# skycrapers/TecoGAN-PyTorch

Hardware: AMD Instinct MI355X
Metric: HR frames/sec/GPU at 4xSR 3x134x320 LR; Vid4 PSNR vs reference (higher is better)
Workload: dtype f32; 1 GPU; TecoGAN 4xSR BD generator-only inference (FRNet.infer_sequence) of a synthetic 2140-frame 3x134x320 LR clip -> 3x536x1280 HR uint8, 1 clip/GPU, random-init weights (BASELINE configs[1]); a step = one recurrent frame; parallelism=clip-sharded x1, no data-path collective, launches_per_frame=29

## Files before the change

### include/tecogan_hip.h

```cpp
#ifndef TECOGAN_HIP_H
#define TECOGAN_HIP_H

#include <stddef.h>
#include <stdint.h>

#ifdef __cplusplus
extern "C" {
#endif

typedef void* tg_stream_t;

enum {
  TG_OK = 0,
  TG_E_SHAPE = -1,
  TG_E_ARG = -2,
  TG_E_HIP = -3
};

enum {
  TG_ACT_NONE = 0,
  TG_ACT_RELU = 1,
  TG_ACT_LRELU02 = 2,
  TG_ACT_TANH24 = 3
};

enum {
  TG_UP_NONE = 0,
  TG_UP_BICUBIC = 1,
  TG_UP_BILINEAR = 2
};

#define TG_ABI_MAJOR 2
int tg_version(void);
const char* tg_last_error_string(void);
const char* tg_build_info(void);

int tg_conv3x3_pick_ocb(int cout);
size_t tg_conv3x3_packed_floats(int cin, int cout, int ocb);
int tg_conv3x3_pack(const float* w, float* w_packed, int cin, int cout, int ocb,
                    int transposed, tg_stream_t stream);

int tg_conv3x3_fwd(
    const float* x, int64_t x_nstride, int c1,
    const float* x2, int64_t x2_nstride,
    const float* w_packed, int ocb, const float* bias ,
    const float* res, int64_t res_nstride,
    float* y, int64_t y_nstride,
    int n, int cin, int cout, int h, int w, int act, tg_stream_t stream);

int tg_conv3x3_fwd_phased(const float* x, int64_t x_nstride, const float* w_packed, int ocb,
                          const float* bias, float* y, int64_t y_nstride, int n, int cin,
                          int cout, int h, int w, int act, int tapsel, int cphase,
                          int taps_phase0, int taps_phase1, tg_stream_t stream);
int tg_conv4x4s2_supported(int n, int ci, int co, int h, int w);
size_t tg_conv4x4s2_packed_floats(int ci, int co);
int tg_conv4x4s2_pack(const float* w, float* w_fwd, float* w_dgrad, int ci, int co, tg_stream_t stream);
size_t tg_conv4x4s2_workspace_floats(int n, int ci, int co, int h, int w, int dgrad);
int tg_conv4x4s2_fwd(const float* x, const float* w_fwd, float* y, float* workspace, int n, int ci, int co, int h, int w,
                     tg_stream_t stream);
int tg_conv4x4s2_dgrad(const float* g, const float* w_dgrad, const float* act_y, int act, float* dx, float* workspace,
                       int n, int ci, int co, int h, int w, tg_stream_t stream);
int tg_conv3x3s2_supported(int n, int cin, int cout, int h_out, int w_out);
int tg_conv3x3s2_fwd(const float* x, int64_t x_nstride, const float* w_packed, const float* bias,
                     const float* relu_mask, int64_t mask_nstride, float* y, int64_t y_nstride, int n,
                     int cin, int cout, int h_out, int w_out, int act, tg_stream_t stream);
int tg_conv3x3_fwd_phased_masked(const float* x, int64_t x_nstride, const float* w_packed, int ocb,
                                 const float* bias, const float* relu_mask, int64_t mask_nstride,
                                 float* y, int64_t y_nstride, int n, int cin, int cout, int h, int w,
                                 int act, int tapsel, int cphase, int taps_phase0, int taps_phase1,
                                 tg_stream_t stream);
int tg_conv3x3_phased_pick_ksplit(int n, int cin, int cout, int h, int w, int ocb);
int tg_conv3x3_fwd_phased_splitk(const float* x, int64_t x_nstride, const float* w_packed, int ocb,
                                 const float* bias, float* y, int n, int cin, int cout, int h, int w,
                                 int act, int tapsel, int cphase, int taps_phase0, int taps_phase1,
                                 int ksplit, float* partials, tg_stream_t stream);
int tg_conv3x3_fwd_masked(const float* x, int64_t x_nstride, int c1, const float* x2,
                          int64_t x2_nstride, const float* w_packed, int ocb,
                          const float* bias, const float* res, int64_t res_nstride,
                          const float* relu_mask, int64_t mask_nstride, float* y,
                          int64_t y_nstride, int n, int cin, int cout, int h, int w, int act,
                          tg_stream_t stream);

int64_t tg_conv3x3_wino_packed_floats(int cin, int cout);
int tg_conv3x3_prefers_wino(int n, int cin, int cout, int h, int w);
int tg_pack_conv3x3_wino(const float* w, float* out, int cin, int cout, int transposed,
                         tg_stream_t stream);
int tg_conv3x3_wino_fwd(const float* x, int64_t x_nstride, int c1, const float* x2,
                        int64_t x2_nstride, const float* u_packed, const float* bias,
                        const float* res, int64_t res_nstride, const float* relu_mask,
                        int64_t mask_nstride, float* y, int64_t y_nstride, int n, int cin,
                        int cout, int h, int w, int act, tg_stream_t stream);

typedef struct {
  const float* x; const float* x2; const float* u_packed; const float* bias; const float* res;
  float* y;
  int64_t x_nstride, x2_nstride, res_nstride, y_nstride;
  int c1, cin, act;
} tg_wino_layer;
int64_t tg_conv3x3_wino_chain_flag_ints(int n_layers, int n, int h, int w);
int tg_conv3x3_wino_chain(const tg_wino_layer* layers, int n_layers, int n, int cout, int h, int w,
                          int32_t* flags, int epoch, tg_stream_t stream);

int tg_conv3x3_wino_resident_supported(int n, int cout, int h, int w);
int64_t tg_conv3x3_wino_resident_ws_bytes(int h, int w);
int tg_conv3x3_wino_resident(const tg_wino_layer* layers, int n_layers, int cout, int h, int w,
                             void* workspace, int epoch, tg_stream_t stream);
typedef struct tg_wres_convt {
  const float* u_packed;
  const float* bias;
  float* y;
  int act;
} tg_wres_convt;
size_t tg_conv3x3_wino_resident_ct_floats(void);
int tg_conv3x3_wino_resident_ct_pack(const float* w_iohw, float* out, tg_stream_t stream);
int tg_conv3x3_wino_resident_ct(const tg_wino_layer* layers, int n_layers, int cout, int h, int w,
                                void* workspace, int epoch, const tg_wres_convt* convt, tg_stream_t stream);

typedef struct {
  const float* x; const float* x2; const float* w_packed; const float* bias; const float* res;
  const float* relu_mask;
  float* y;
  int64_t x_nstride, x2_nstride, res_nstride, mask_nstride, y_nstride;
  int c1, cin, cout, act;
} tg_chain_layer;
int64_t tg_conv3x3_chain_flag_ints(int n_layers, int n, int h, int w);
int tg_conv3x3_chain_supported(int n, int h, int w, int cmax);
size_t tg_conv3x3_pack16_floats(void);
int tg_conv3x3_pack16(const float* w, float* w_packed, int cin, int cout, int transposed, tg_stream_t stream);
typedef struct tg_pack_item {
  const float* w;
  float* out;
  int cin, cout, transposed, i_total, i_off;
} tg_pack_item;
size_t tg_conv3x3_chain_packed_floats(int pack_layout, int cin);
int tg_conv3x3_chain_pack(const tg_pack_item* items, int n_items, int pack_layout, tg_stream_t stream);
int tg_conv3x3_chain(const tg_chain_layer* layers, int n_layers, int n, int h, int w, int pack_layout,
                     int32_t* flags, int32_t* err, uint32_t epoch, int poll_limit, tg_stream_t stream);
typedef struct { const float* w; const float* b; } tg_packed_layer;
int tg_srnet_body_fwd(const tg_packed_layer* layers, int pack_layout, int nb, const float* lr, int c_lr,
                      const float* tran, int c_tran, float* acts, int n, int nf, int h, int w, int32_t* flags,
                      int32_t* err, uint32_t epoch, int poll_limit, tg_stream_t stream);
int tg_srnet_body_bwd(const tg_packed_layer* dgrad, int pack_layout, int nb, const float* acts, float* dz,
                      float* d_tran, int c_tran, int n, int nf, int h, int w, int32_t* flags, int32_t* err,
                      uint32_t epoch, int poll_limit, tg_stream_t stream);

size_t tg_wgrad3x3_body_workspace_floats(int nframes, int n_per_frame, int nlayers, int c, int h, int w);
int tg_wgrad3x3_body(const float* const* dz_bases, const float* const* act_bases, int nframes, int64_t layer_stride, int nlayers, float* const* grads, float* workspace,
                     int n_per_frame, int c, int h, int w, int accumulate, tg_stream_t stream);
int tg_wgrad3x3_body_bias(const float* const* dz_bases, const float* const* act_bases, int nframes,
                          int64_t layer_stride, int nlayers, float* const* grads, float* const* dbs,
                          float* workspace, int n_per_frame, int c, int h, int w, int accumulate,
                          tg_stream_t stream);
int tg_bias_grad_body(const float* const* dz_bases, int nframes,
                      int64_t layer_stride, int nlayers, float* const* dbs, int n_per_frame, int c, int hw,
                      tg_stream_t stream);

int tg_conv3x3_pick_ksplit(int n, int cin, int cout, int h, int w);
int tg_conv3x3_splitk_fwd(const float* x, int64_t x_nstride, int c1, const float* x2,
                          int64_t x2_nstride, const float* w_packed, int ocb,
                          const float* bias, float* y, int n, int cin, int cout, int h,
                          int w, int act, int ksplit, float* partials, int pool,
                          tg_stream_t stream);

int tg_convt3x3s2_fwd(const float* x, int64_t x_nstride, const float* w_packed,
                      const float* bias, float* y, int64_t y_nstride, int n,
                      int cin, int cout, int h, int w, int act,
                      tg_stream_t stream);
int tg_convt_pack_wz(const float* w_out_oihw, float* wz, int cz, int nf, tg_stream_t stream);
int tg_convt3x3s2_z_fwd(const float* x, int64_t x_nstride, const float* w_packed,
                        const float* bias, const float* wz, int cz, float* z,
                        int64_t z_nstride, int n, int cin, int cout, int h, int w, int act,
                        tg_stream_t stream);
int tg_convt3x3s2_z_fwd_form(const float* x, int64_t x_nstride, const float* w_packed,
                             const float* bias, const float* wz, int cz, float* z,
// ... 281 lines not shown
```

### tecogan-pytorch_amd/_lib.py

```python
import ctypes as C
import os

_HERE = os.path.dirname(os.path.abspath(__file__))
LIB_PATH = os.environ.get('TECOGAN_HIP_LIB') or os.path.join(_HERE, 'libtecogan_hip.so')

TG_OK = 0
ABI_MAJOR = 2
ACT_NONE, ACT_RELU, ACT_LRELU02, ACT_TANH24 = 0, 1, 2, 3
UP_NONE, UP_BICUBIC, UP_BILINEAR = 0, 1, 2
PREC_F32, PREC_F16 = 0, 1

P, I, I64, F, SZ = C.c_void_p, C.c_int, C.c_int64, C.c_float, C.c_size_t


class FrnetCfg(C.Structure):
    _fields_ = [(k, C.c_int) for k in
                ('in_nc', 'out_nc', 'nf', 'nb', 'scale', 'up_mode', 'n', 'h', 'w', 'fnet_only')]


class WinoLayer(C.Structure):
    _fields_ = [('x', C.c_void_p), ('x2', C.c_void_p), ('u_packed', C.c_void_p), ('bias', C.c_void_p),
                ('res', C.c_void_p), ('y', C.c_void_p), ('x_nstride', C.c_int64), ('x2_nstride', C.c_int64),
                ('res_nstride', C.c_int64), ('y_nstride', C.c_int64), ('c1', C.c_int), ('cin', C.c_int),
                ('act', C.c_int)]
# ... 63 lines not shown
    'tg_psnr_sse_u8': (I, [P, P, P, I, I, I, I, P]),
    'tg_luma_u8': (I, [P, P, I64, P]),
    'tg_lpips_conv_fwd': (I, [P, P, I, P, P, P, P, I, I, I, I, I, I, I, I, P]),
    'tg_maxpool3s2_fwd': (I, [P, P, I, I, I, P]),
    'tg_lpips_head_workspace_bytes': (I64, [I, I, I]),
    'tg_lpips_head': (I, [P, P, P, I, I, I, I, P, P, I, P, P]),
    'tg_ssim_workspace_bytes': (I64, [I, I, I]),
    'tg_ssim_y_u8': (I, [P, P, I, I, I, I, I, I, I, I, I, P, P, SZ, P]),
    'tg_psnr_yfloat_partials': (I64, [I, I]),
    'tg_psnr_yfloat_sse_u8': (I, [P, P, I, I, I, I, I, I, I, I, I, P, P]),
    'tg_wgrad3x3_workspace_floats': (SZ, [I, I, I, I, I]),
    'tg_wgrad3x3': (I, [P, I64, P, I64, P, P, I, I, I, I, I, I, I, I, P]),
    'tg_wgrad3x3_multi': (I, [P, P, I, I64, I64, P, P, I, I, I, I, I, I, I, I, P]),
    'tg_wgrad3x3_multi_bias': (I, [P, P, I, I64, I64, P, P, P, I, I, I, I, I, I, I, I, P]),
    'tg_wgrad3x3_multi_phased': (I, [P, P, I, I64, I64, P, P, I, I, I, I, I, I, I, I, I, P]),
    'tg_conv3x3_phased_pick_ksplit': (I, [I, I, I, I, I, I]),
    'tg_conv3x3_fwd_phased_splitk': (I, [P, I64, P, I, P, P, I, I, I, I, I, I, I, I, I, I, I, P, P]),
    'tg_wgrad3x3_convt_workspace_floats': (SZ, [I, I, I, I, I]),
    'tg_wgrad3x3_convt_multi': (I, [P, P, I, P, P, P, I, I, I, I, I, I, P]),
    'tg_bias_grad_multi': (I, [P, I, P, I, I, I, I, P]),
    'tg_act_bwd': (I, [P, P, P, I64, I, P]),
    'tg_bias_grad': (I, [P, P, I, I, I, I, P]),
    'tg_maxpool2_bwd': (I, [P, P, P, I, I, I, P]),
    'tg_upsample_bwd': (I, [P, P, I, I, I, I, I, F, P]),
    'tg_backward_warp_bwd': (I, [P, P, P, P, P, I, I, I, I, P]),
    'tg_backward_warp_bwd_acc': (I, [P, P, P, P, P, I, I, I, I, P]),
    'tg_conv3x3_wino_resident_ct_floats': (SZ, []),
    'tg_conv3x3_wino_resident_ct_pack': (I, [P, P, P]),
    'tg_conv3x3_wino_resident_ct': (I, [P, I, I, I, I, P, I, P, P]),
    'tg_conv4x4s2_supported': (I, [I, I, I, I, I]),
    'tg_conv4x4s2_packed_floats': (SZ, [I, I]),
    'tg_conv4x4s2_pack': (I, [P, P, P, I, I, P]),
    'tg_conv4x4s2_workspace_floats': (SZ, [I, I, I, I, I, I]),
    'tg_conv4x4s2_fwd': (I, [P, P, P, P, I, I, I, I, I, P]),
    'tg_conv4x4s2_dgrad': (I, [P, P, P, I, P, P, I, I, I, I, I, P]),
    'tg_backward_warp_s2d_fwd': (I, [P, P, P, I, I, I, I, I, P]),
    'tg_backward_warp_s2d_bwd': (I, [P, P, P, P, I, P, I, I, I, I, I, P]),
    'tg_depth_to_space': (I, [P, P, I, I, I, I, I, P]),
    'tg_depth_to_space_act_bwd_supported': (I, [P, P, P, I, I]),
    'tg_depth_to_space_act_bwd': (I, [P, P, I, P, I, I, I, I, I, P]),
    'tg_charbonnier': (I, [P, P, I64, F, F, P, F, P, P]),
    'tg_channel_norm': (I, [P, P, P, P, I, I, I64, P]),
    'tg_cosine_loss': (I, [P, P, I, I, I64, F, F, P, F, P, P]),
    'tg_pixel_loss': (I, [P, P, I64, I, F, P, F, P, P]),
    'tg_bce_logits': (I, [P, I64, F, F, P, F, P, P]),
    'tg_lsgan_loss': (I, [P, I64, F, F, P, F, P, P]),
    'tg_adam_step': (I, [P, P, P, P, I64, F, F, F, F, F, I, P]),
    'tg_adam_step_guarded': (I, [P, P, P, P, I64, F, F, F, F, F, I, P, P]),
    'tg_fault_to_slot': (I, [P, P, P]),
    'tg_axpy': (I, [P, P, F, I64, P]),
    'tg_div_scalar': (I, [P, P, F, I64, P]),
    'tg_bn_lrelu_train_fwd': (I, [P, P, P, P, P, F, F, F, P, P, P, I, I, I, P]),
    'tg_bn_lrelu_train_bwd': (I, [P, P, P, P, P, P, F, P, P, P, I, P, I, I, I, P]),
    'tg_bn_local_stats': (I, [P, P, I, I, I, P]),
    'tg_bn_merge_stats': (I, [P, I, F, F, F, P, P, P, P, I, P]),
    'tg_bn_lrelu_apply': (I, [P, P, P, P, P, F, P, I, I, I, P]),
    'tg_bn_lrelu_bwd_reduce': (I, [P, P, P, P, P, F, P, I, I, I, P]),
    'tg_bn_lrelu_bwd_apply': (I, [P, P, P, P, P, P, P, F, F, P, I, I, I, P]),
    'tg_linear1_fwd': (I, [P, P, P, P, I, I, P]),
    'tg_linear1_bwd': (I, [P, P, P, P, P, P, I, I, I, P]),
    'tg_downsample_bd': (I, [P, P, P, I, I, I, I, I, I, P]),
    'tg_conv3x3_wino_packed_floats': (I64, [I, I]),
    'tg_conv3x3_wino_chain_flag_ints': (I64, [I, I, I, I]),
    'tg_conv3x3_wino_chain': (I, [C.POINTER(WinoLayer), I, I, I, I, I, P, I, P]),
    'tg_conv3x3_wino_resident_supported': (I, [I, I, I, I]),
    'tg_conv3x3_wino_resident_ws_bytes': (I64, [I, I]),
    'tg_conv3x3_wino_resident': (I, [C.POINTER(WinoLayer), I, I, I, I, P, I, P]),
    'tg_conv3x3_chain_flag_ints': (I64, [I, I, I, I]),
    'tg_conv3x3_chain_supported': (I, [I, I, I, I]),
    'tg_conv3x3_pack16_floats': (SZ, []),
    'tg_conv3x3_pack16': (I, [P, P, I, I, I, P]),
    'tg_conv3x3_chain_packed_floats': (SZ, [I, I]),
    'tg_conv3x3_chain_pack': (I, [P, I, I, P]),
    'tg_conv3x3_chain': (I, [C.POINTER(ChainLayer), I, I, I, I, I, P, P, C.c_uint32, I, P]),
    'tg_srnet_body_fwd': (I, [C.POINTER(PackedLayer), I, I, P, I, P, I, P, I, I, I, I, P, P, C.c_uint32, I, P]),
    'tg_srnet_body_bwd': (I, [C.POINTER(PackedLayer), I, I, P, P, P, I, I, I, I, I, P, P, C.c_uint32, I, P]),
    'tg_wgrad3x3_body_workspace_floats': (SZ, [I, I, I, I, I, I]),
    'tg_wgrad3x3_body': (I, [P, P, I, I64, I, P, P, I, I, I, I, I, P]),
    'tg_wgrad3x3_body_bias': (I, [P, P, I, I64, I, P, P, P, I, I, I, I, I, P]),
    'tg_bias_grad_body': (I, [P, I, I64, I, P, I, I, I, P]),
    'tg_conv3x3_prefers_wino': (I, [I, I, I, I, I]),
    'tg_pack_conv3x3_wino': (I, [P, P, I, I, I, P]),
    'tg_conv3x3_wino_fwd': (I, [P, I64, I, P, I64, P, P, P, I64, P, I64, P, I64, I, I, I, I, I, I, P]),
    'tg_time_gather': (I, [P, P, P, I, I, I, I64, P]),
    'tg_transpose01': (I, [P, P, I, I, I64, P]),
    'tg_stack_time': (I, [P, I, P, I, I64, P]),
    'tg_index_gather': (I, [P, P, P, I64, I64, I, P]),
    'tg_pingpong_grad': (I, [P, P, I, I, I64, P]),
    'tg_d_assemble_fwd': (I, [P, I, P, P, I, P, I, I, I, I, I, I, I, P]),
    'tg_d_assemble_bwd': (I, [P, P, I, P, I, I, I, I, I, I, I, P]),
    'tg_gather_clips_u8': (I, [P, P, P, P, I, I, I, I, P]),
    'tg_comm_get_unique_id': (I, [P]),
    'tg_comm_init_rank': (I, [P, I, I, C.POINTER(C.c_void_p)]),
    'tg_comm_destroy': (I, [P]),
    'tg_comm_world': (I, [P]),
    'tg_comm_rank': (I, [P]),
    'tg_comm_query': (I, [P, C.POINTER(C.c_int), C.POINTER(C.c_int)]),
    'tg_comm_library_origin': (C.c_char_p, []),
    'tg_allreduce_sum_f32': (I, [P, P, I64, P]),
    'tg_allgather_f32': (I, [P, P, P, I64, P]),
    'tg_frnet_workspace_floats': (SZ, [C.POINTER(FrnetCfg)]),
    'tg_frnet_plan_create': (I, [C.POINTER(FrnetCfg), C.POINTER(LayerWeights), I, P,
                                 C.POINTER(C.c_void_p)]),
    'tg_frnet_plan_destroy': (None, [P]),
    'tg_frnet_plan_chain_status': (I, [P, C.POINTER(C.c_int), C.POINTER(C.c_int)]),
    'tg_frnet_plan_set_chain_poll_limit': (I, [P, I]),
    'tg_frnet_plan_set_chain_rearm': (I, [P, I]),
    'tg_frnet_plan_chain_rearms': (I, [P, P, P]),
    'tg_frnet_plan_hold_chain_rearm': (I, [P, I]),
    'tg_frnet_step': (I, [P, P, P, P, P, P, P]),
    'tg_frnet_step_phase': (I, [P, I, I, P, P, P, P, P, P]),
    'tg_frnet_plan_launches': (I, [P]),
    'tg_frnet_plan_flow': (P, [P, I]),
    'tg_frnet_step_srnet': (I, [P, P, P, P, P, P, P]),
    'tg_frnet_plan_kinds': (I, []),
    'tg_frnet_kind_name': (C.c_char_p, [I]),
    'tg_frnet_plan_kind_stats': (I, [P, I, C.POINTER(C.c_int), C.POINTER(C.c_double),
                                     C.POINTER(C.c_double)]),
    'tg_frnet_replay': (I, [P, P, P, P, P, C.c_uint, I, P]),
    'tg_frnet_step_masked': (I, [P, P, P, P, P, P, C.c_uint, P]),
    'tg_conv3x3_f16_supported': (I, [I, I, I, I, I]),
    'tg_conv3x3_f16_packed_halves': (SZ, [I, I]),
    'tg_conv3x3_f16_act_halves': (I64, [I, I, I]),
    'tg_conv3x3_f16_pack_weights': (I, [P, I, I, I, P, P]),
    'tg_conv3x3_f16_pack_input': (I, [P, I64, I, P, I64, I, P, I, I, I, P]),
    'tg_conv3x3_f16_fwd': (I, [P, P, P, P, P, I, I, I, I, I, I, P]),
    'tg_convt3x3s2_f16_fwd': (I, [P, P, P, P, I64, I, I, I, I, I, I, P]),
    'tg_frnet_f16_workspace_bytes': (SZ, [C.POINTER(FrnetCfg)]),
    'tg_frnet_plan_set_precision': (I, [P, I, C.POINTER(LayerWeights), I, P]),
    'tg_frnet_plan_precision': (I, [P]),
}

_lib = None


class TecoganHipError(RuntimeError):
    pass


def lib():
    global _lib
    if _lib is None:
        if not os.path.isfile(LIB_PATH):
            raise TecoganHipError(
                f'{LIB_PATH} not found: build it with '
                f'`bash {os.path.join(_HERE, "csrc", "build.sh")}` '
                '(hipcc --offload-arch=gfx950).  There is no CPU/ATen fallback.')
        import torch
        handle = C.CDLL(LIB_PATH)
        handle.tg_version.restype = I
        if handle.tg_version() // 100 != ABI_MAJOR:
            raise TecoganHipError(f'{LIB_PATH}: ABI {handle.tg_version()} but this binding is written for '
                                  f'major {ABI_MAJOR} (include/tecogan_hip.h TG_ABI_MAJOR): rebuild the library')
        for name, (res, args) in SIGNATURES.items():
            fn = getattr(handle, name)
            fn.restype = res
            fn.argtypes = args
        _lib = handle
    return _lib


def check(rc, what):
    if rc != TG_OK:
        msg = lib().tg_last_error_string().decode('utf-8', 'replace')
        raise TecoganHipError(f'{what} failed (code {rc}): {msg}')
```

### tecogan-pytorch_amd/csrc/tg_api.hip

```cpp
#include <new>
#include <vector>

#include "tg_common.h"

namespace tg {
static thread_local char g_err[512] = "ok";
void set_error(const char* fmt, ...) {
  va_list ap;
  va_start(ap, fmt);
  vsnprintf(g_err, sizeof(g_err), fmt, ap);
  va_end(ap);
}
}

extern "C" int tg_version(void) { return TG_ABI_MAJOR * 100 + 1; }
extern "C" const char* tg_last_error_string(void) { return tg::g_err; }

#ifndef TG_BUILD_FLAGS_STR
#define TG_BUILD_FLAGS_STR "unknown (not built by csrc/build.sh)"
#endif
#ifndef TG_FILE_FLAGS_STR
#define TG_FILE_FLAGS_STR ""
#endif
namespace tg { int wres_lab_bits(); }
// ... 143 lines not shown

extern "C" size_t tg_frnet_workspace_floats(const tg_frnet_cfg* cfg) {
  if (!cfg_ok(cfg)) return 0;
  size_t off[15];
  carve(cfg, off);
  return off[14];
}

extern "C" int tg_frnet_plan_create(const tg_frnet_cfg* cfg, const tg_layer_weights* layers,
                                    int n_layers, float* workspace, tg_frnet_plan** out) {
  TG_REQUIRE(cfg && layers && workspace && out, TG_E_ARG, "frnet_plan_create: null pointer");
  TG_REQUIRE(cfg_ok(cfg), TG_E_SHAPE,
             "frnet_plan_create: unsupported cfg (in_nc=3, out_nc<=4, nf<=64, scale 2|4, h,w>=8)");
  int nup = cfg->scale == 4 ? 2 : 1;
  int need = 14 + 1 + 2 * cfg->nb + nup + 1;
  TG_REQUIRE(n_layers == need, TG_E_ARG, "frnet_plan_create: %d layers given, %d expected",
             n_layers, need);
  for (int i = 0; i < n_layers; ++i)
    TG_REQUIRE(layers[i].w && layers[i].b, TG_E_ARG, "frnet_plan_create: layer %d null", i);
  tg_frnet_plan* p = new (std::nothrow) tg_frnet_plan();
  TG_REQUIRE(p, TG_E_ARG, "frnet_plan_create: out of host memory");
  p->cfg = *cfg;
  p->L.assign(layers, layers + n_layers);
  size_t off[15];
  carve(cfg, off);
  p->f16 = false; p->f16_ready = false; p->HWT = p->HA = p->HB = nullptr;
  p->WZ = workspace + off[11]; p->wz_ready = false;
  p->WA = p->WZ + 2048; p->wa_ready = false;
  p->RESWS = workspace + off[13]; p->res_ready = false;
  p->CHAINF = reinterpret_cast<int32_t*>(workspace + off[12]); p->chain_ready = false; p->epoch = 0; p->chain_layers = 0;
  p->chain_err = nullptr; p->chain_disabled = false; p->chain_faults = 0; p->chain_poll_limit = tg::TG_CHAIN_POLL_LIMIT_DEFAULT;
  p->rearm_first = 64; p->rearm_wait = 0; p->clean_frames = 0; p->rearms = 0; p->rearm_fence = nullptr; p->fence_set = false;
  p->rearm_hold = false;
  if (!cfg->fnet_only) {
    void* hp = nullptr;
    if (hipHostMalloc(&hp, 64, hipHostMallocMapped | hipHostMallocCoherent) == hipSuccess && hp) {
      p->chain_err = static_cast<int32_t*>(hp);
      for (int i = 0; i < 16; ++i) p->chain_err[i] = 0;
    } else {
      (void)hipGetLastError();
    }
  }
  p->FA = workspace + off[7]; p->FB = workspace + off[8]; p->FPART = workspace + off[9];
  p->FLOW2 = workspace + off[10];
  p->PART = workspace + off[6];
  p->A = workspace + off[0]; p->B = workspace + off[1]; p->FLOW = workspace + off[2];
  p->S2D = workspace + off[3]; p->U1 = workspace + off[4];
  p->U2 = cfg->scale == 4 ? workspace + off[5] : nullptr;
  p->fh = cfg->h / 8 * 8; p->fw = cfg->w / 8 * 8;
  account(p);
  *out = p;
  return TG_OK;
}

extern "C" void tg_frnet_plan_destroy(tg_frnet_plan* plan) {
  if (!plan) return;
  if (plan->chain_err) (void)hipHostFree(plan->chain_err);
  if (plan->rearm_fence) (void)hipEventDestroy(plan->rearm_fence);
  delete plan;
}
extern "C" int tg_frnet_plan_launches(const tg_frnet_plan* plan) { return plan ? plan->launches : 0; }

enum {
  K_CONV64_R2 = 0,
  K_CONV64_R4 = 1,
  K_CONV32 = 2,
  K_CONVT = 3,
  K_SMALL = 4,
  K_WARP = 5,
  K_POOL = 6,
  K_UPSAMPLE = 7,
  K_QUANT = 8,
  K_FINAL = 9,
  K_CONV64_KS = 10,
  K_CONVT_Z = 11,
  K_TAIL = 12,
  K_CONV_ONESHOT = 13,
  K_CONV_WINO = 14,
  K_WINO_CHAIN = 15,
  K_WINO_RES = 16,
  K_F16_PACK = 17,
  K_F16_CONV = 18,
  K_F16_CONVT = 19,
  K_COUNT = 20
};

static bool hr_fuse_enabled() {
  static const int v = TG_LAB_ENV("TG_HR_FUSE", 1);
  return v != 0;
}
static bool convtz_wino_enabled() {
  static const int v = TG_LAB_ENV("TG_CONVTZ_WINO", 1);
  return v != 0;
}
static bool chain_wanted(long long ntile) {
  static const int v = [] { const char* e = getenv("TG_WINO_CHAIN"); return e && *e ? atoi(e) : -1; }();
  if (v >= 0) return v != 0;
  return ntile > 768 && ntile <= 3000;
}
static bool resident_wanted(bool layer_prefers_wino) {
  static const int v = [] { const char* e = getenv("TG_WINO_RES"); return e && *e ? atoi(e) : -1; }();
  return v >= 0 ? v != 0 : layer_prefers_wino;
}
static bool plan_u8_ok(const tg_frnet_plan* p) {
  if (p->f16 && p->cfg.scale == 2) return p->cfg.n == 1;
  return p->cfg.n == 1 || (hr_fuse_enabled() && p->cfg.out_nc <= 3 && p->cfg.nf <= 64);
}

static int step_impl(tg_frnet_plan* p, const float* lr_curr, const float* lr_prev,
                     const float* hr_prev, float* hr_out, uint8_t* u8_out, tg_stream_t st,
                     unsigned mask, bool dry, int phases, int slot, const float* flow_ext) {
  const tg_frnet_cfg& c = p->cfg;
  float* const flow_buf = flow_ext ? const_cast<float*>(flow_ext) : (slot ? p->FLOW2 : p->FLOW);
  bool active = (phases & 1) != 0;
  float* part_buf = p->FPART;
  const int n = c.n, h = c.h, w = c.w, s = c.scale;
  const int64_t hw = (int64_t)h * w;
  int li = 0;
  float *A = p->FA, *B = p->FB;
  int rc = TG_OK;
  if (!dry && (phases & 2) && mask == 0xFFFFFFFFu) chain_rearm_tick(p, st);
  auto go = [&](int kind, double flops, double bytes, auto&& fn) {
    if (rc != TG_OK) return;
    if (dry) {
      p->st_launch[kind] += 1; p->st_flops[kind] += flops; p->st_bytes[kind] += bytes;
      return;
    }
    if (active && (mask & (1u << kind))) rc = fn();
  };
  auto conv = [&](const float* x, int64_t xns, int c1, const float* x2, int64_t x2ns, int cin,
                  int cout, int hh, int ww, int act, const float* res, int64_t rns, float* y,
                  int64_t yns, bool pool = false, float* pool_tmp = nullptr) {
    const tg_layer_weights lw = p->L[li++];
    int ocb = tg_conv3x3_pick_ocb(cout);
    int kind = ocb == 32 ? K_CONV32
                         : (tg::conv3x3_rows_per_wg(ocb, (long long)n * hh * ww) == 4 ? K_CONV64_R4
                                                                                       : K_CONV64_R2);
    double px = (double)n * hh * ww;
    double fl = 2.0 * cin * 9 * cout * px;
    double by = 4.0 * px * (cin + cout + (res ? cout : 0)) + 4.0 * 9 * cin * cout;
    if (lw.u && tg_conv3x3_prefers_wino(n, cin, cout, hh, ww)) {
      float* yw = pool ? pool_tmp : y;
      go(K_CONV_WINO, fl, by, [&] {
        return tg::conv3x3_wino_launch(x, xns, c1, x2, x2ns, lw.u, lw.b, res, rns, nullptr, 0, yw,
                                       pool ? (int64_t)cout * hh * ww : yns, n, cin, cout, hh, ww, act, st);
      });
      if (pool)
        go(K_POOL, 0, 4.0 * n * cout * (hh * ww + (hh / 2) * (ww / 2)),
           [&] { return tg_maxpool2_fwd(yw, y, n * cout, hh, ww, st); });
      return;
    }
    int ks = res ? 1 : tg_conv3x3_pick_ksplit(n, cin, cout, hh, ww);
    if (ks == 1 && kind == K_CONV64_R2 && tg::conv3x3_uses_wg_ksplit(n, cin, cout, hh, ww))
      kind = tg::conv3x3_uses_oneshot(n, cin, cout, hh, ww) ? K_CONV_ONESHOT : K_CONV64_KS;
    if (ks > 1) {
      go(kind, fl, by, [&] {
        return tg::conv3x3_splitk_conv(x, xns, c1, x2, x2ns, lw.w, ocb, n, cin, cout, hh, ww, ks,
                                       part_buf, st);
      });
      go(K_FINAL, 0, 4.0 * px * cout * (ks + 1), [&] {
        return tg::conv3x3_splitk_finalize(part_buf, ks, lw.b, act, pool ? 1 : 0, y, n, cout, hh, ww,
                                           st);
      });
      return;
    }
    float* yc = pool ? pool_tmp : y;
    go(kind, fl, by, [&] {
      return tg_conv3x3_fwd(x, xns, c1, x2, x2ns, lw.w, ocb, lw.b, res, rns, yc,
                            pool ? (int64_t)cout * hh * ww : yns, n, cin, cout, hh, ww, act, st);
    });
    if (pool)
      go(K_POOL, 0, 4.0 * n * cout * (hh * ww + (hh / 2) * (ww / 2)),
         [&] { return tg_maxpool2_fwd(yc, y, n * cout, hh, ww, st); });
  };
  int hh = h, ww = w;
  const int enc[3] = {32, 64, 128};
  int cin = 2 * c.in_nc;
  const float* src = nullptr;
  for (int e = 0; e < 3; ++e) {
    int co = enc[e];
    if (e == 0)
      conv(lr_curr, c.in_nc * hw, c.in_nc, lr_prev, c.in_nc * hw, cin, co, hh, ww, TG_ACT_LRELU02,
           nullptr, 0, A, (int64_t)co * hh * ww);
    else
      conv(src, (int64_t)cin * hh * ww, cin, nullptr, 0, cin, co, hh, ww, TG_ACT_LRELU02, nullptr,
           0, A, (int64_t)co * hh * ww);
    conv(A, (int64_t)co * hh * ww, co, nullptr, 0, co, co, hh, ww, TG_ACT_LRELU02, nullptr, 0, A,
         (int64_t)co * (hh / 2) * (ww / 2), true, B);
    hh /= 2; ww /= 2; cin = co;
    float* t = A; A = B; B = t;
    src = B;
  }
  const int dec[3] = {256, 128, 64};
  for (int d = 0; d < 3; ++d) {
    int co = dec[d];
    conv(src, (int64_t)cin * hh * ww, cin, nullptr, 0, cin, co, hh, ww, TG_ACT_LRELU02, nullptr, 0,
         A, (int64_t)co * hh * ww);
    conv(A, (int64_t)co * hh * ww, co, nullptr, 0, co, co, hh, ww, TG_ACT_LRELU02, nullptr, 0, B,
         (int64_t)co * hh * ww);
    {
      float *pi = B, *po = A; int ph = hh, pw = ww;
      go(K_UPSAMPLE, 0, 4.0 * n * co * ph * pw * 5.0,
         [&] { return tg_upsample_fwd(pi, po, n * co, ph, pw, 2, TG_UP_BILINEAR, 1.0f, st); });
    }
    hh *= 2; ww *= 2; cin = co;
    float* t = A; A = B; B = t;
    src = B;
  }
  conv(src, (int64_t)cin * hh * ww, cin, nullptr, 0, cin, 32, hh, ww, TG_ACT_LRELU02, nullptr, 0, A,
       (int64_t)32 * hh * ww);
  {
    const tg_layer_weights lw = p->L[li++];
    float* ai = A; int fh_ = hh, fw_ = ww;
    go(K_SMALL, 2.0 * 32 * 9 * 2 * n * fh_ * fw_, 4.0 * n * fh_ * fw_ * 34, [&] {
      return tg_conv3x3_small_fwd(ai, (int64_t)32 * fh_ * fw_, lw.w, lw.b, nullptr, TG_UP_NONE, 1,
                                  flow_buf, (int64_t)2 * fh_ * fw_, n, 32, 2, fh_, fw_,
                                  TG_ACT_TANH24, st);
    });
  }
  active = (phases & 2) != 0;
  part_buf = p->PART;
  const int s2dc = s * s * c.in_nc;
  go(K_WARP, 0,
     4.0 * n * ((double)c.in_nc * s * s * hw * 2 + 2.0 * p->fh * p->fw), [&] {
       return tg_flowup_warp_s2d_fwd(flow_buf, p->fh, p->fw, hr_prev, p->S2D, s2dc * hw, nullptr, n,
                                     c.in_nc, h, w, s, c.up_mode, st);
     });
  A = p->A; B = p->B;
  const int nf = c.nf;
  const bool in_wino = p->L[li].u && tg_conv3x3_prefers_wino(n, c.in_nc + s2dc, nf, h, w);
  const int skip = in_wino ? 0 : 1;
  const int nchain = 1 + 2 * c.nb - skip;
  bool chain = p->chain_err && !p->chain_disabled && nf <= 64 && nchain >= 2 && nchain <= CHAIN_MAX_LAYERS &&
               chain_wanted((long long)n * tg::cdiv(h, 2) * tg::cdiv(w, 32)) &&
               tg_conv3x3_prefers_wino(n, nf, nf, h, w);
  for (int i = skip; i < 1 + 2 * c.nb && chain; ++i) chain = p->L[li + i].u != nullptr;
  bool resident = p->chain_err && !p->chain_disabled && n == 1 && nchain >= 2 && nchain <= CHAIN_MAX_LAYERS &&
                  resident_wanted(tg_conv3x3_prefers_wino(n, nf, nf, h, w) != 0) && (skip || c.in_nc + s2dc <= 64) && tg::conv3x3_wino_resident_ok(n, nf, h, w);
  for (int i = skip; i < 1 + 2 * c.nb && resident; ++i) resident = p->L[li + i].u != nullptr && p->L[li + i].b != nullptr;
  if (resident) chain = true;
  bool ct_fold = false;
  if (p->f16) {
    const int nbody = 1 + 2 * c.nb;
    const size_t wstep = tg_conv3x3_f16_packed_halves(64, 64);
    if (!dry && !p->f16_ready && (phases & 2)) {
      for (int k = 0; k <= nbody && rc == TG_OK; ++k)
        rc = tg_conv3x3_f16_pack_weights(p->HL[k].w, k == 0 ? c.in_nc + s2dc : nf, nf, k == nbody ? 1 : 0,
                                         p->HWT + k * wstep, st);
      p->f16_ready = rc == TG_OK;
    }
    const double px = (double)n * h * w;
    const double lfl = 2.0 * nf * 9 * nf * px, lby = 2.0 * px * 2 * nf + 2.0 * 9 * nf * nf;
    uint16_t *HA = p->HA, *HB = p->HB;
    go(K_F16_PACK, 0, px * (4.0 * (c.in_nc + s2dc) + 2.0 * 64), [&] {
      return tg_conv3x3_f16_pack_input(lr_curr, c.in_nc * hw, c.in_nc, p->S2D, s2dc * hw, s2dc, HB, n, h, w, st);
    });
    auto hconv = [&](int k, const uint16_t* xin, const uint16_t* res, uint16_t* y, int act) {
      go(K_F16_CONV, lfl, lby + (res ? 2.0 * px * nf : 0), [&] {
        return tg_conv3x3_f16_fwd(xin, p->HWT + k * wstep, p->HL[k].b, res, y, n, 64, 64, h, w, act, st);
      });
    };
    hconv(0, HB, nullptr, HA, TG_ACT_RELU);
    for (int b = 0; b < c.nb; ++b) {
      hconv(1 + 2 * b, HA, nullptr, HB, TG_ACT_RELU);
      hconv(2 + 2 * b, HB, HA, HA, TG_ACT_NONE);
    }
    go(K_F16_CONVT, lfl, 2.0 * px * nf + 4.0 * px * nf * 4 + 2.0 * 9 * nf * nf, [&] {
      return tg_convt3x3s2_f16_fwd(HA, p->HWT + nbody * wstep, p->HL[nbody].b, p->U1, (int64_t)nf * 4 * hw, n, 64, 64,
                                   h, w, TG_ACT_RELU, st);
    });
    li += nbody;
    ct_fold = true;
  } else if (chain) {
    if (skip)
      conv(lr_curr, c.in_nc * hw, c.in_nc, p->S2D, s2dc * hw, c.in_nc + s2dc, nf, h, w, TG_ACT_RELU,
           nullptr, 0, A, nf * hw);
    tg_wino_layer cl[CHAIN_MAX_LAYERS];
    double fl = 0, by = 0;
    const double px = (double)n * h * w;
    for (int k = 0; k < nchain; ++k) {
      const int i = k + skip;
      const tg_layer_weights lw = p->L[li + k];
      tg_wino_layer& d = cl[k];
      const bool first = i == 0, conv2 = !first && (i % 2 == 0);
      d.x = first ? lr_curr : (conv2 ? B : A);
      d.x2 = first ? p->S2D : nullptr;
      d.u_packed = lw.u; d.bias = lw.b;
      d.res = conv2 ? A : nullptr;
      d.y = (first || conv2) ? A : B;
      d.x_nstride = first ? c.in_nc * hw : nf * hw;
      d.x2_nstride = first ? s2dc * hw : 0;
      d.res_nstride = nf * hw; d.y_nstride = nf * hw;
      d.c1 = first ? c.in_nc : nf;
// ... 178 lines not shown
  TG_REQUIRE(p, TG_E_ARG, "frnet_plan_chain_status: null plan");
  const int rc = chain_poll(p);
  if (faults_total) *faults_total = p->chain_faults;
  if (chain_active) *chain_active = (p->chain_layers > 0 && !p->chain_disabled) ? 1 : 0;
  return rc;
}

extern "C" int tg_frnet_plan_set_chain_poll_limit(tg_frnet_plan* p, int poll_limit) {
  TG_REQUIRE(p, TG_E_ARG, "frnet_plan_set_chain_poll_limit: null plan");
  p->chain_poll_limit = poll_limit;
  return TG_OK;
}

extern "C" int tg_frnet_plan_set_chain_rearm(tg_frnet_plan* p, int first_after_frames) {
  TG_REQUIRE(p && first_after_frames >= 0, TG_E_ARG, "frnet_plan_set_chain_rearm: bad argument");
  p->rearm_first = first_after_frames;
  if (p->chain_disabled && p->rearm_wait == 0) p->rearm_wait = first_after_frames;
  return TG_OK;
}

extern "C" int tg_frnet_plan_hold_chain_rearm(tg_frnet_plan* p, int hold) {
  TG_REQUIRE(p, TG_E_ARG, "frnet_plan_hold_chain_rearm: null plan");
  p->rearm_hold = hold != 0;
  return TG_OK;
}

extern "C" int tg_frnet_plan_chain_rearms(const tg_frnet_plan* p, int* rearms, int* current_wait_frames) {
  TG_REQUIRE(p, TG_E_ARG, "frnet_plan_chain_rearms: null plan");
  if (rearms) *rearms = p->rearms;
  if (current_wait_frames) *current_wait_frames = p->rearm_wait;
  return TG_OK;
}

extern "C" size_t tg_frnet_f16_workspace_bytes(const tg_frnet_cfg* cfg) {
  if (!cfg_ok(cfg) || cfg->fnet_only || cfg->nf != 64) return 0;
  const size_t wbytes = (size_t)(2 + 2 * cfg->nb) * tg_conv3x3_f16_packed_halves(64, 64) * 2;
  const size_t abytes = (size_t)tg_conv3x3_f16_act_halves(cfg->n, cfg->h, cfg->w) * 2;
  return align64(wbytes) + 2 * align64(abytes);
}

extern "C" int tg_frnet_plan_set_precision(tg_frnet_plan* p, int precision, const tg_layer_weights* plain,
                                           int n_plain, void* workspace) {
  TG_REQUIRE(p, TG_E_ARG, "frnet_plan_set_precision: null plan");
  TG_REQUIRE(precision == TG_PREC_F32 || precision == TG_PREC_F16, TG_E_ARG,
             "frnet_plan_set_precision: precision %d (TG_PREC_F32 | TG_PREC_F16)", precision);
  if (precision == TG_PREC_F16) {
    const tg_frnet_cfg& c = p->cfg;
    TG_REQUIRE(!c.fnet_only, TG_E_ARG, "frnet_plan_set_precision: an FNet-only plan has no SRNet body");
    TG_REQUIRE(c.nf == 64 && tg_conv3x3_f16_supported(c.n, 64, 64, c.h, c.w), TG_E_ARG,
               "frnet_plan_set_precision: the fp16 body needs nf = 64 (nf = %d)", c.nf);
    TG_REQUIRE(plain && n_plain == 2 + 2 * c.nb, TG_E_ARG, "frnet_plan_set_precision: %d plain layers given, %d expected",
               n_plain, 2 + 2 * c.nb);
    for (int i = 0; i < n_plain; ++i)
      TG_REQUIRE(plain[i].w && plain[i].b, TG_E_ARG, "frnet_plan_set_precision: plain layer %d null", i);
    TG_REQUIRE(workspace && (reinterpret_cast<uintptr_t>(workspace) & 15) == 0, TG_E_ARG,
               "frnet_plan_set_precision: workspace null or not 16-byte aligned");
    p->HL.assign(plain, plain + n_plain);
    const size_t wbytes = align64((size_t)n_plain * tg_conv3x3_f16_packed_halves(64, 64) * 2);
    const size_t abytes = align64((size_t)tg_conv3x3_f16_act_halves(c.n, c.h, c.w) * 2);
    unsigned char* base = static_cast<unsigned char*>(workspace);
    p->HWT = reinterpret_cast<uint16_t*>(base);
    p->HA = reinterpret_cast<uint16_t*>(base + wbytes);
    p->HB = reinterpret_cast<uint16_t*>(base + wbytes + abytes);
    p->f16_ready = false;
  }
  p->f16 = precision == TG_PREC_F16;
  p->res_ready = false; p->chain_ready = false;
  account(p);
  return TG_OK;
}

extern "C" int tg_frnet_plan_precision(const tg_frnet_plan* p) { return p && p->f16 ? TG_PREC_F16 : TG_PREC_F32; }

extern "C" int tg_frnet_plan_kinds(void) { return K_COUNT; }

extern "C" const char* tg_frnet_kind_name(int kind) {
  static const char* names[K_COUNT] = {
      "conv3x3_mfma_kernel<2,2,1>", "conv3x3_mfma_kernel<4,1,2>", "conv3x3_mfma_kernel<4,1,1>",
      "convt3x3s2_mfma_kernel",      "conv3x3_small_kernel",       "flowup_warp_s2d_kernel",
      "maxpool2_kernel",             "upsample_kernel",            "quantize_u8_hwc_kernel",
      "splitk_finalize_kernel",      "conv3x3_mfma_kernel<1,2,1,KS=2>",
      "convt3x3s2_mfma_kernel<Z>",   "convout_tail_kernel",        "conv3x3_oneshot_kernel",
      "conv3x3_wino_kernel",         "conv3x3_wino_chain_kernel",  "conv3x3_wino_resident_kernel",
      "pack_input_f16_kernel",       "conv3x3_f16_kernel<false>",  "conv3x3_f16_kernel<true>"};
  return (kind >= 0 && kind < K_COUNT) ? names[kind] : "?";
}

extern "C" int tg_frnet_plan_kind_stats(const tg_frnet_plan* p, int kind, int* launches,
                                        double* flops, double* bytes) {
  TG_REQUIRE(p && kind >= 0 && kind < K_COUNT, TG_E_ARG, "plan_kind_stats: bad argument");
  if (launches) *launches = p->st_launch[kind];
  if (flops) *flops = p->st_flops[kind];
  if (bytes) *bytes = p->st_bytes[kind];
  return TG_OK;
}
```

### tecogan-pytorch_amd/csrc/tg_common.h

```cpp
#pragma once
#include <hip/hip_runtime.h>
#include <stdarg.h>
#include <stdint.h>
#include <stdio.h>

#include <stdlib.h>

#include "../../include/tecogan_hip.h"

#ifndef TG_LAB
#define TG_LAB 0
#endif
#if TG_LAB
#define TG_LAB_ENV(name, dflt) ([] { const char* e_ = getenv(name); return e_ ? atoi(e_) : (dflt); }())
#else
#define TG_LAB_ENV(name, dflt) (dflt)
#endif

namespace tg {

void set_error(const char* fmt, ...);

inline int check_launch(const char* what) {
  hipError_t e = hipGetLastError();
  if (e != hipSuccess) {
    set_error("%s: %s", what, hipGetErrorString(e));
    return TG_E_HIP;
  }
  return TG_OK;
}

#define TG_REQUIRE(cond, code, ...) \
  do {                              \
    if (!(cond)) {                  \
      tg::set_error(__VA_ARGS__);   \
      return (code);                \
    }                               \
  } while (0)

bool convt_z_split_rule(int n, int h, int w, int form);
bool convt_z_wino_split_rule(int n, int h, int w, int split);

int conv3x3_splitk_conv(const float* x, int64_t x_nstride, int c1, const float* x2,
                        int64_t x2_nstride, const float* w_packed, int ocb, int n, int cin,
                        int cout, int h, int w, int ksplit, float* partials, tg_stream_t stream);
int conv3x3_splitk_finalize(const float* partials, int ksplit, const float* bias, int act, int pool,
                            float* y, int n, int cout, int h, int w, tg_stream_t stream);

inline int conv3x3_rows_per_wg(int ocb, long long pixels) {
  if (ocb == 32) return 4;
  return pixels >= 200000 ? 4 : 2;
}

__host__ __device__ inline int cdiv(int a, int b) { return (a + b - 1) / b; }

bool conv3x3_uses_wg_ksplit(int n, int cin, int cout, int h, int w);
bool conv3x3_uses_oneshot(int n, int cin, int cout, int h, int w);
int conv3x3_wino_launch(const float* x, int64_t x_ns, int c1, const float* x2, int64_t x2_ns, const float* u,
                        const float* bias, const float* res, int64_t res_ns, const float* mask,
                        int64_t mask_ns, float* y, int64_t y_ns, int n, int cin, int cout, int h, int w,
                        int act, tg_stream_t stream);

constexpr int TG_CHAIN_POLL_LIMIT_DEFAULT = 1 << 21;
int conv3x3_wino_chain_launch(const tg_wino_layer* layers, int n_layers, int n, int cout, int h, int w,
                              int32_t* flags, int32_t* err, unsigned epoch, int poll_limit, tg_stream_t stream);

bool conv3x3_wino_resident_ok(int n, int cout, int h, int w);
int64_t conv3x3_wino_resident_ws_bytes(int h, int w);
int conv3x3_wino_resident_launch(const tg_wino_layer* layers, int n_layers, int cout, int h, int w, void* ws,
                                 int32_t* err, unsigned base, int poll_limit, tg_stream_t stream,
                                 const tg_wres_convt* ct = nullptr);

typedef float f32x16 __attribute__((ext_vector_type(16)));
typedef float f32x4 __attribute__((ext_vector_type(4)));

constexpr int CK = 8;

__device__ __forceinline__ float apply_act(float v, int act) {
  switch (act) {
    case TG_ACT_RELU: return v > 0.f ? v : 0.f;
    case TG_ACT_LRELU02: return v >= 0.f ? v : v * 0.2f;
    case TG_ACT_TANH24: return tanhf(v) * 24.f;
    default: return v;
  }
}

__device__ __forceinline__ float act_slope(int act) {
  return act == TG_ACT_RELU ? 0.f : (act == TG_ACT_LRELU02 ? 0.2f : 1.f);
}

inline float act_slope_host(int act) {
  return act == TG_ACT_RELU ? 0.f : (act == TG_ACT_LRELU02 ? 0.2f : 1.f);
}

__device__ __forceinline__ void bicubic_w(int d, int f, float k[4]) {
  const float a = -0.75f;
  float s = (float)d / (float)f;
  float s2 = s * s, s3 = s2 * s;
  k[0] = ((0.f * 1.f + a * s) + (-2.f * a) * s2) + a * s3;
  k[1] = ((1.f * 1.f + 0.f * s) + (-(a + 3.f)) * s2) + (a + 2.f) * s3;
  k[2] = ((0.f * 1.f + (-a) * s) + (2.f * a + 3.f) * s2) + (-(a + 2.f)) * s3;
  k[3] = ((0.f * 1.f + 0.f * s) + a * s2) + (-a) * s3;
}

__device__ __forceinline__ void bilinear_src(int dst, int scale, int in_size,
                                             int& i0, int& i1, float& l0,
                                             float& l1) {
  float src = ((float)dst + 0.5f) * (1.0f / (float)scale) - 0.5f;
  src = src < 0.f ? 0.f : src;
  i0 = (int)floorf(src);
  i1 = i0 + 1 < in_size ? i0 + 1 : in_size - 1;
  l1 = src - (float)i0;
  l0 = 1.0f - l1;
}

__device__ __forceinline__ float linspace_m1p1(int i, int n, float step) {
  const int mirror = n - 1 - i;
  const int j = i < mirror ? i : mirror;
  const unsigned flip = (unsigned)(n / 2 - 1 - i) & 0x80000000u;
  return __builtin_bit_cast(float, __builtin_bit_cast(unsigned, __builtin_fmaf(step, (float)j, -1.0f)) ^ flip);
}

__device__ __forceinline__ float warp_coord(int i, int n, float flow) {
  float step = 2.0f / (float)(n - 1);
  float half = (float)(n - 1) / 2.0f;
  float g = linspace_m1p1(i, n, step) + flow / half;
  float p = (g + 1.0f) * half;
  p = __builtin_fmaxf(p, 0.f);
  p = __builtin_fminf(p, (float)(n - 1));
  return p;
}

}
```

### tecogan-pytorch_amd/csrc/tg_conv3x3_mfma.hip

```cpp
#include "tg_common.h"
#include <cstdlib>

namespace tg {

constexpr int TW = 32;
constexpr int PW = TW + 2;
constexpr int RS = 34;

struct Conv3x3Args {
  const float* x;
  const float* x2;
  const float* wpk;
  const float* bias;
  const float* res;
  float* y;
  long long x_ns, x2_ns, res_ns, y_ns;
  int c1, cin, cout, h, w, act;
  int tiles_x, tiles_y, nchunk, nocg;
  int ksplit;
  float* part;
  long long part_ss;
  int vec_ok;
  long long* dbg;
  int nblocks;
  const float* mask;
  long long mask_ns;
  int tapsel, cphase;
  unsigned char rowsets[2];
};

__global__ void pack3x3_kernel(const float* __restrict__ w, float* __restrict__ out,
                               int cin, int cout, int ocb, int nchunk, int nocg,
                               int transposed) {
  int total = nocg * nchunk * 9 * CK * ocb;
  for (int i = blockIdx.x * blockDim.x + threadIdx.x; i < total;
       i += gridDim.x * blockDim.x) {
    int j = i & 3;
    int t = i >> 2;
    int o = t % ocb; t /= ocb;
    int half = t & 1; t >>= 1;
    int tap = t % 9; t /= 9;
    int ch = t % nchunk;
    int g = t / nchunk;
    int oc = g * ocb + o, ci = ch * CK + 4 * half + j;
    float v = 0.f;
    if (oc < cout && ci < cin) {
      if (transposed == 2) v = w[((size_t)ci * cout + oc) * 9 + (8 - tap)];
      else if (transposed == 1) v = w[((size_t)ci * cout + oc) * 9 + tap];
      else v = w[((size_t)oc * cin + ci) * 9 + tap];
    }
    out[i] = v;
  }
}

__device__ __forceinline__ float buf_load(__amdgpu_buffer_rsrc_t r, unsigned voff) {
  return __builtin_bit_cast(float, __builtin_amdgcn_raw_buffer_load_b32(r, (int)voff, 0, 0));
}

constexpr unsigned OOB = 0x80000000u;

enum { TAPS_ALL = 0, TAPS_01 = 1, TAPS_12 = 2, TAPS_1 = 3 };
__host__ __device__ constexpr int taps_first(int code) { return (code == TAPS_12 || code == TAPS_1) ? 1 : 0; }
__host__ __device__ constexpr int taps_count(int code) { return code == TAPS_ALL ? 3 : (code == TAPS_1 ? 1 : 2); }

template <int NT, int OCB, int RY, int RX>
__device__ __forceinline__ void chunk_taps(const float* si, const float* sw, f32x16 (&acc)[NT]) {
  constexpr int Y0 = taps_first(RY), NY = taps_count(RY), X0 = taps_first(RX), NX = taps_count(RX);
  constexpr int N = NY * NX;
  f32x4 bq[2], aq[2][NT];
  auto fetch = [&](int i, int slot) {
    const int ky = Y0 + i / NX, kx = X0 + i % NX;
    bq[slot] = *reinterpret_cast<const f32x4*>(si + (ky * 2 * 34 + kx) * 4);
#pragma unroll
    for (int t = 0; t < NT; ++t)
      aq[slot][t] = *reinterpret_cast<const f32x4*>(sw + (ky * 3 + kx) * (2 * OCB * 4) + t * 128);
  };
  fetch(0, 0);
#pragma unroll
  for (int i = 0; i < N; ++i) {
    const int cur = i & 1;
    if (i + 1 < N) fetch(i + 1, cur ^ 1);
#pragma unroll
    for (int kk = 0; kk < 4; ++kk) {
#pragma unroll
      for (int t = 0; t < NT; ++t)
        acc[t] = __builtin_amdgcn_mfma_f32_32x32x2f32(aq[cur][t][kk], bq[cur][kk], acc[t], 0, 0, 0);
    }
  }
}

template <int NT, int OCB>
__device__ __forceinline__ void chunk_taps_sel(int ry, int rx, const float* si, const float* sw,
                                               f32x16 (&acc)[NT]) {
  switch (ry * 4 + rx) {
    case TAPS_01 * 4 + TAPS_01: chunk_taps<NT, OCB, TAPS_01, TAPS_01>(si, sw, acc); break;
    case TAPS_01 * 4 + TAPS_12: chunk_taps<NT, OCB, TAPS_01, TAPS_12>(si, sw, acc); break;
    case TAPS_12 * 4 + TAPS_01: chunk_taps<NT, OCB, TAPS_12, TAPS_01>(si, sw, acc); break;
    case TAPS_12 * 4 + TAPS_12: chunk_taps<NT, OCB, TAPS_12, TAPS_12>(si, sw, acc); break;
    case TAPS_01 * 4 + TAPS_1: chunk_taps<NT, OCB, TAPS_01, TAPS_1>(si, sw, acc); break;
    case TAPS_1 * 4 + TAPS_01: chunk_taps<NT, OCB, TAPS_1, TAPS_01>(si, sw, acc); break;
    case TAPS_1 * 4 + TAPS_1: chunk_taps<NT, OCB, TAPS_1, TAPS_1>(si, sw, acc); break;
    case TAPS_12 * 4 + TAPS_1: chunk_taps<NT, OCB, TAPS_12, TAPS_1>(si, sw, acc); break;
    case TAPS_1 * 4 + TAPS_12: chunk_taps<NT, OCB, TAPS_1, TAPS_12>(si, sw, acc); break;
    default: chunk_taps<NT, OCB, TAPS_ALL, TAPS_ALL>(si, sw, acc); break;
  }
}

template <int WM, int WN, int NT, bool DUAL, int ABL = 0, int KS = 1>
__global__ __launch_bounds__(WM* WN* KS * 64) void conv3x3_mfma_kernel(Conv3x3Args a) {
  static_assert(KS == 1 || KS == 2, "wave groups over K: one or two");
  constexpr int NTHREADS = WM * WN * KS * 64;
  constexpr int OCB = WN * NT * 32;
  constexpr int PH = WM + 2;
  constexpr int IN_ITEMS = PH * 2 * PW;
  constexpr int IN_FLOATS = PH * 2 * RS * 4;
  constexpr int W_FLOATS = 9 * CK * OCB;
  constexpr int I_PER_T = (IN_ITEMS + NTHREADS - 1) / NTHREADS;

  extern __shared__ __attribute__((aligned(16))) float smem[];
  float* s_in = smem;
  float* s_w = smem + 2 * KS * IN_FLOATS;

  const int tid = threadIdx.x;
  const int lane = tid & 63;
  const int wave = tid >> 6;
  const int wm = wave % WM;
  const int wn = (wave / WM) % WN;
  const int wk = wave / (WM * WN);
  auto bufof = [](int ch) { return KS == 1 ? (ch & 1) : ((ch >> 1) & 1); };

  int b = blockIdx.x;
  if (a.nblocks > 0) {
    const int per = (a.nblocks + 7) >> 3;
    b = (b & 7) * per + (b >> 3);
    if (b >= a.nblocks) return;
  }
  const int tx = b % a.tiles_x; b /= a.tiles_x;
  const int ty = b % a.tiles_y; b /= a.tiles_y;
  const int ocg = b % a.nocg; b /= a.nocg;
  const int ks = b % a.ksplit;
  const int n = b / a.ksplit;
  const int x0 = tx * TW, y0 = ty * WM;
  const int hw = a.h * a.w;
  const int ch_begin = (int)((long long)ks * a.nchunk / a.ksplit);
  const int ch_end = (int)((long long)(ks + 1) * a.nchunk / a.ksplit);

  unsigned voff[I_PER_T];
  int lds_item[I_PER_T];
#pragma unroll
  for (int i = 0; i < I_PER_T; ++i) {
    int q = tid + i * NTHREADS;
    int r = q / (2 * PW), rem = q - r * (2 * PW);
    int hf = rem / PW, col = rem - hf * PW;
    int gy = y0 - 1 + r, gx = x0 - 1 + col;
    bool ok = q < IN_ITEMS && gy >= 0 && gy < a.h && gx >= 0 && gx < a.w;
    voff[i] = ok ? (unsigned)((4 * hf * hw + gy * a.w + gx) * 4) : OOB;
    lds_item[i] = q < IN_ITEMS ? ((r * 2 + hf) * RS + col) * 4 : -1;
  }
  const __amdgpu_buffer_rsrc_t rs1 = __builtin_amdgcn_make_buffer_rsrc(
      const_cast<float*>(a.x + (long long)n * a.x_ns), 0, a.c1 * hw * 4, 0x00020000);
  const __amdgpu_buffer_rsrc_t rs2 = __builtin_amdgcn_make_buffer_rsrc(
      const_cast<float*>(DUAL ? a.x2 + (long long)n * a.x2_ns : a.x), 0,
      DUAL ? (a.cin - a.c1) * hw * 4 : 0, 0x00020000);
  const unsigned plane = (unsigned)hw * 4u;

  const f32x4* wsrc =
      reinterpret_cast<const f32x4*>(a.wpk + (size_t)ocg * a.nchunk * W_FLOATS);

  f32x4 rin[KS][I_PER_T];

  auto load_chunk = [&](int ch) {
    if (!((ABL & 32) && ch != ch_begin))
#pragma unroll
    for (int k = 0; k < KS; ++k) {
      const unsigned cbase = (unsigned)((ch + k) * CK) * plane;
#pragma unroll
      for (int i = 0; i < I_PER_T; ++i) {
#pragma unroll
        for (int j = 0; j < 4; ++j) {
          unsigned o1 = voff[i] + cbase + (unsigned)j * plane;
          float v = buf_load(rs1, o1);
          if (DUAL) v += buf_load(rs2, o1 - (unsigned)a.c1 * plane);
          rin[k][i][j] = v;
        }
      }
    }
    if ((ABL & 64) && ch != ch_begin) return;
    constexpr int PIECES = W_FLOATS * 4 / 1024;
    constexpr int NWAVES = NTHREADS / 64;
    const char* src = reinterpret_cast<const char*>(wsrc + (size_t)ch * (W_FLOATS / 4)) + lane * 16;
    char* dst = reinterpret_cast<char*>(s_w + bufof(ch) * KS * W_FLOATS);
    const int valid = (ch_end - ch < KS ? ch_end - ch : KS) * PIECES;
#pragma unroll
    for (int i = 0; i < (KS * PIECES + NWAVES - 1) / NWAVES; ++i) {
      int piece = wave + i * NWAVES;
      if (piece < valid)
        __builtin_amdgcn_global_load_lds(
            (const __attribute__((address_space(1))) void*)(src + piece * 1024),
            (__attribute__((address_space(3))) void*)(dst + piece * 1024), 16, 0, 0);
    }
  };
  auto store_chunk = [&](int buf) {
#pragma unroll
    for (int k = 0; k < KS; ++k) {
      float* si = s_in + (buf * KS + k) * IN_FLOATS;
#pragma unroll
      for (int i = 0; i < I_PER_T; ++i)
        if (lds_item[i] >= 0) *reinterpret_cast<f32x4*>(si + lds_item[i]) = rin[k][i];
    }
  };

  f32x16 acc[NT];
#pragma unroll
  for (int t = 0; t < NT; ++t)
#pragma unroll
    for (int r = 0; r < 16; ++r) acc[t][r] = 0.f;

  const int lh = lane >> 5, ll = lane & 31;
  const int b_off = ((wm * 2 + lh) * RS + ll) * 4;
  const int a_off = (lh * OCB + wn * (NT * 32) + ll) * 4;

  long long tk0 = 0, tk1 = 0, t_mfma = 0, t_sync = 0, t_issue = 0;
  if constexpr (ABL & 16) tk0 = clock64();
  load_chunk(ch_begin);
  store_chunk(bufof(ch_begin));
  __syncthreads();
  if constexpr (ABL & 16) tk1 = clock64();

  for (int ch = ch_begin; ch < ch_end; ch += KS) {
    long long ta = 0, tb = 0, tc = 0;
    if constexpr (ABL & 16) ta = clock64();
    const int buf = bufof(ch);
    const bool more = (ch + KS < ch_end) && !(ABL & 1);
    if (more) load_chunk(ch + KS);

    if constexpr (ABL & 16) tb = clock64();
    const float* si = s_in + (buf * KS + wk) * IN_FLOATS + b_off;
    const float* sw = s_w + (buf * KS + wk) * W_FLOATS + a_off;
    if (KS == 1 || ch + wk < ch_end) {
    if (a.tapsel) {
      const int ph = a.tapsel == 1 ? ((ch + wk) * CK) / a.cphase : (ocg * OCB) / a.cphase;
      chunk_taps_sel<NT, OCB>(a.rowsets[(ph >> 1) & 1], a.rowsets[ph & 1], si, sw, acc);
    } else {
    f32x4 bq[2], aq[2][NT];
    bq[0] = *reinterpret_cast<const f32x4*>(si);
#pragma unroll
    for (int t = 0; t < NT; ++t) aq[0][t] = *reinterpret_cast<const f32x4*>(sw + t * 128);
#pragma unroll
    for (int tap = 0; tap < 9; ++tap) {
      const int cur = tap & 1, nxt = cur ^ 1;
      if (tap + 1 < 9 && !(ABL & 8)) {
        const int ky = (tap + 1) / 3, kx = (tap + 1) % 3;
        bq[nxt] = *reinterpret_cast<const f32x4*>(si + (ky * 2 * RS + kx) * 4);
#pragma unroll
        for (int t = 0; t < NT; ++t)
          aq[nxt][t] = *reinterpret_cast<const f32x4*>(sw + (tap + 1) * (2 * OCB * 4) + t * 128);
      }
#pragma unroll
      for (int kk = 0; kk < 4; ++kk) {
#pragma unroll
        for (int t = 0; t < NT; ++t)
          acc[t] = __builtin_amdgcn_mfma_f32_32x32x2f32(aq[cur][t][kk], bq[cur][kk], acc[t], 0, 0, 0);
      }
    }
    }
    }
    if constexpr (ABL & 16) {
      asm volatile("s_nop 0" ::"v"(acc[0][0]));
      tc = clock64();
    }
    if (more) store_chunk(buf ^ 1);
    if (!(ABL & 2)) __syncthreads();
    if constexpr (ABL & 16) {
      long long td = clock64();
      t_issue += tb - ta; t_mfma += tc - tb; t_sync += td - tc;
    }
  }
  if constexpr (ABL & 16) {
    if (a.dbg && tid == 0) {
      long long* d = a.dbg + (long long)blockIdx.x * 8;
      d[0] = tk0; d[1] = tk1 - tk0; d[2] = t_issue; d[3] = t_mfma; d[4] = t_sync; d[5] = clock64();
      d[6] = __builtin_amdgcn_s_getreg((20 << 0) | (0 << 6) | ((4 - 1) << 11));
    }
  }

  if constexpr (KS == 2) {
    float* red = smem;
    if (wk == 1) {
#pragma unroll
      for (int t = 0; t < NT; ++t)
#pragma unroll
        for (int r = 0; r < 16; ++r)
          red[(((wn * WM + wm) * NT + t) * 16 + r) * 64 + lane] = acc[t][r];
    }
    __syncthreads();
    if (wk == 0) {
#pragma unroll
      for (int t = 0; t < NT; ++t)
#pragma unroll
        for (int r = 0; r < 16; ++r)
          acc[t][r] += red[(((wn * WM + wm) * NT + t) * 16 + r) * 64 + lane];
    }
    __syncthreads();
  }
  const bool do_ep = wk == 0;
  const int px = x0 + ll, py = y0 + wm;
  const bool inimg = px < a.w && py < a.h;
  const long long opix = (long long)py * a.w + px;
  const int ocb0 = ocg * OCB + wn * (NT * 32) + 4 * lh;
  if (a.ksplit > 1) {
    if (inimg) {
      float* pb = a.part + (long long)ks * a.part_ss + (long long)n * a.cout * hw + opix;
#pragma unroll
      for (int t = 0; t < NT; ++t)
#pragma unroll
        for (int r = 0; r < 16; ++r) {
          int oc = ocb0 + t * 32 + (r & 3) + 8 * (r >> 2);
          if (oc < a.cout) pb[(long long)oc * hw] = acc[t][r];
        }
    }
    return;
  }
  const float slope = act_slope(a.act);
  if (a.vec_ok) {
    constexpr int ES = 36;
    float* ep = smem + (wave % (WM * WN)) * (NT * 32 * ES);
    if (do_ep) {
#pragma unroll
      for (int t = 0; t < NT; ++t)
#pragma unroll
        for (int r = 0; r < 16; ++r)
          ep[(t * 32 + (r & 3) + 8 * (r >> 2) + 4 * lh) * ES + ll] = acc[t][r];
    }
    __syncthreads();
    const int ocw = ocg * OCB + wn * (NT * 32);
    if (do_ep && py < a.h) {
#pragma unroll
      for (int j = 0; j < NT * 4; ++j) {
        int idx4 = j * 64 + lane;
        int ol = idx4 >> 3, p4 = (idx4 & 7) * 4;
        int oc = ocw + ol;
        int gx = x0 + p4;
        if (oc < a.cout && gx < a.w) {
          f32x4 v = *reinterpret_cast<const f32x4*>(ep + ol * ES + p4);
          float bb = a.bias ? a.bias[oc] : 0.f;
          long long off = (long long)oc * hw + (long long)py * a.w + gx;
          f32x4 rr = {0.f, 0.f, 0.f, 0.f};
          if (a.res) rr = *reinterpret_cast<const f32x4*>(a.res + (long long)n * a.res_ns + off);
          f32x4 mm = {1.f, 1.f, 1.f, 1.f};
          if (a.mask) mm = *reinterpret_cast<const f32x4*>(a.mask + (long long)n * a.mask_ns + off);
#pragma unroll
          for (int e = 0; e < 4; ++e) {
            float q = v[e] + bb;
            q = (q >= 0.f ? q : q * slope + 0.f) + rr[e];
            v[e] = mm[e] > 0.f ? q : 0.f;
          }
          *reinterpret_cast<f32x4*>(a.y + (long long)n * a.y_ns + off) = v;
        }
      }
    }
    return;
  }
  if (!do_ep) return;
  float bv[NT][16], rv[NT][16];
  unsigned dead[NT];
#pragma unroll
  for (int t = 0; t < NT; ++t) dead[t] = 0u;
#pragma unroll
  for (int t = 0; t < NT; ++t)
#pragma unroll
    for (int r = 0; r < 16; ++r) {
      int oc = ocb0 + t * 32 + (r & 3) + 8 * (r >> 2);
      int occ = oc < a.cout ? oc : a.cout - 1;
      bv[t][r] = a.bias ? a.bias[occ] : 0.f;
      rv[t][r] = (a.res && inimg) ? a.res[(long long)n * a.res_ns + opix + (long long)occ * hw] : 0.f;
      if (a.mask && inimg && a.mask[(long long)n * a.mask_ns + opix + (long long)occ * hw] <= 0.f)
        dead[t] |= 1u << r;
    }
  if (inimg) {
    float* yb = a.y + (long long)n * a.y_ns + opix;
#pragma unroll
    for (int t = 0; t < NT; ++t)
#pragma unroll
      for (int r = 0; r < 16; ++r) {
        int oc = ocb0 + t * 32 + (r & 3) + 8 * (r >> 2);
        float v = acc[t][r] + bv[t][r];
        v = (v >= 0.f ? v : v * slope + 0.f) + rv[t][r];
        if (dead[t] & (1u << r)) v = 0.f;
        if (oc < a.cout && (!(ABL & 4) || v == 12345.678f)) yb[(long long)oc * hw] = v;
      }
  }
}

template <bool DUAL>
__global__ __launch_bounds__(512) void conv3x3_oneshot_kernel(Conv3x3Args a) {
  constexpr int OCB = 64, KG = 4, MAXCH = 8;
  constexpr int IN_FLOATS = 3 * 2 * RS * 4;
  constexpr int ITEMS_PER_CH = 3 * 2 * PW;
  constexpr int W_VEC4 = 9 * CK * OCB / 4;
  extern __shared__ __attribute__((aligned(16))) float smem[];
  float* s_in = smem;
  float* red = smem + MAXCH * IN_FLOATS;

  const int tid = threadIdx.x, lane = tid & 63, wave = tid >> 6;
  const int wn = wave & 1, wk = wave >> 1;
  const int lh = lane >> 5, ll = lane & 31;
  int b = blockIdx.x;
  const int tx = b % a.tiles_x; b /= a.tiles_x;
  const int ty = b % a.tiles_y;
  const int n = b / a.tiles_y;
  const int x0 = tx * TW, y0 = ty;
  const int hw = a.h * a.w;
  const unsigned plane = (unsigned)hw * 4u;
  const int nchunk = a.nchunk;
  const __amdgpu_buffer_rsrc_t rs1 = __builtin_amdgcn_make_buffer_rsrc(
      const_cast<float*>(a.x + (long long)n * a.x_ns), 0, a.c1 * hw * 4, 0x00020000);
  const __amdgpu_buffer_rsrc_t rs2 = __builtin_amdgcn_make_buffer_rsrc(
      const_cast<float*>(DUAL ? a.x2 + (long long)n * a.x2_ns : a.x), 0,
      DUAL ? (a.cin - a.c1) * hw * 4 : 0, 0x00020000);

  const int cpw = (nchunk + KG - 1) / KG;
  const int c0 = wk * cpw;
  const f32x4* wlane = reinterpret_cast<const f32x4*>(a.wpk) + (lh * OCB + wn * 32 + ll);
  f32x4 aw[2][9];
#pragma unroll
  for (int ci = 0; ci < 2; ++ci) {
    const int c = c0 + ci;
    const bool on = ci < cpw && c < nchunk;
#pragma unroll
    for (int tap = 0; tap < 9; ++tap) {
      f32x4 v = {0.f, 0.f, 0.f, 0.f};
      if (on) v = wlane[(size_t)c * W_VEC4 + tap * (2 * OCB)];
      aw[ci][tap] = v;
    }
  }
  const int total = nchunk * ITEMS_PER_CH;
  constexpr int MAXQ = (MAXCH * ITEMS_PER_CH + 511) / 512;
#pragma unroll
  for (int k0 = 0; k0 < MAXQ; k0 += 2) {
    f32x4 v[2];
#pragma unroll
    for (int k = 0; k < 2; ++k) {
      const int q = tid + (k0 + k) * 512;
      const int ch = q / ITEMS_PER_CH, rem = q - ch * ITEMS_PER_CH;
      const int r = rem / (2 * PW), rem2 = rem - r * (2 * PW);
      const int hf = rem2 / PW, col = rem2 - hf * PW;
      const int gy = y0 - 1 + r, gx = x0 - 1 + col;
      const bool ok = q < total && gy >= 0 && gy < a.h && gx >= 0 && gx < a.w;
      const unsigned base = ok ? (unsigned)(((ch * CK + 4 * hf) * hw + gy * a.w + gx) * 4) : OOB;
#pragma unroll
      for (int j = 0; j < 4; ++j) {
        const unsigned o1 = base + (unsigned)j * plane;
        float t = buf_load(rs1, o1);
        if (DUAL) t += buf_load(rs2, o1 - (unsigned)a.c1 * plane);
        v[k][j] = t;
      }
    }
#pragma unroll
    for (int k = 0; k < 2; ++k) {
      const int q = tid + (k0 + k) * 512;
      const int ch = q / ITEMS_PER_CH, rem = q - ch * ITEMS_PER_CH;
      const int r = rem / (2 * PW), rem2 = rem - r * (2 * PW);
      const int hf = rem2 / PW, col = rem2 - hf * PW;
      if (q < total) *reinterpret_cast<f32x4*>(s_in + ch * IN_FLOATS + ((r * 2 + hf) * RS + col) * 4) = v[k];
    }
  }
  __syncthreads();

  f32x16 acc;
#pragma unroll
  for (int r = 0; r < 16; ++r) acc[r] = 0.f;
#pragma unroll
  for (int ci = 0; ci < 2; ++ci) {
    const int c = c0 + ci;
// ... 136 lines not shown
      const float* si = s_in + c * IN_FLOATS + (lh * RS2 + 2 * ll) * 4;
#pragma unroll
      for (int tap = 0; tap < 9; ++tap) {
        const int ky = tap / 3, kx = tap % 3;
        const f32x4 bq = *reinterpret_cast<const f32x4*>(si + (ky * 2 * RS2 + kx) * 4);
#pragma unroll
        for (int kk = 0; kk < 4; ++kk)
          acc = __builtin_amdgcn_mfma_f32_32x32x2f32(aw[ci][tap][kk], bq[kk], acc, 0, 0, 0);
      }
    }
  }
  if (wk > 0) {
#pragma unroll
    for (int r = 0; r < 16; ++r) red[((wn * (KG - 1) + wk - 1) * 16 + r) * 64 + lane] = acc[r];
  }
  __syncthreads();
  constexpr int ES = 36;
  float* ep = smem;
  if (wk == 0) {
#pragma unroll
    for (int g = 0; g < KG - 1; ++g)
#pragma unroll
      for (int r = 0; r < 16; ++r) acc[r] += red[((wn * (KG - 1) + g) * 16 + r) * 64 + lane];
#pragma unroll
    for (int r = 0; r < 16; ++r) ep[(wn * 32 + (r & 3) + 8 * (r >> 2) + 4 * lh) * ES + ll] = acc[r];
  }
  __syncthreads();
  const float slope = act_slope(a.act);
  for (int i = tid; i < 64 * TW; i += 512) {
    const int oc = i >> 5, p = i & 31;
    const int gx = x0 + p;
    if (oc < a.cout && gx < a.w) {
      const long long off = (long long)oc * hw + (long long)y0 * a.w + gx;
      float q = ep[oc * ES + p] + (a.bias ? a.bias[oc] : 0.f);
      q = (q >= 0.f ? q : q * slope + 0.f) + (a.res ? a.res[(long long)n * a.res_ns + off] : 0.f);
      if (a.mask && a.mask[(long long)n * a.mask_ns + off] <= 0.f) q = 0.f;
      a.y[(long long)n * a.y_ns + off] = q;
    }
  }
}


template <int WM, int WN, int NT, int KS = 1>
static int launch_conv(const Conv3x3Args& a0, int n, hipStream_t stream) {
  Conv3x3Args a = a0;
  a.vec_ok = (a.w % 4 == 0) && ((uintptr_t)a.y % 16 == 0) && (a.y_ns % 4 == 0) &&
             (!a.res || (((uintptr_t)a.res % 16 == 0) && (a.res_ns % 4 == 0))) &&
             (!a.mask || (((uintptr_t)a.mask % 16 == 0) && (a.mask_ns % 4 == 0)));
  constexpr int OCB = WN * NT * 32;
  a.tiles_x = cdiv(a.w, TW);
  a.tiles_y = cdiv(a.h, WM);
  a.nocg = cdiv(a.cout, OCB);
  a.nchunk = cdiv(a.cin, CK);
  size_t lds = 2 * KS * (size_t)((WM + 2) * 2 * RS * 4 + 9 * CK * OCB) * sizeof(float);
  if (a.ksplit < 1) a.ksplit = 1;
  TG_REQUIRE(KS == 1 || a.ksplit == 1, TG_E_ARG, "conv3x3: in-workgroup K split excludes ksplit");
  if (KS > 1) {
    static bool attr_set = false;
    if (!attr_set) {
      (void)hipFuncSetAttribute(reinterpret_cast<const void*>(
                              conv3x3_mfma_kernel<WM, WN, NT, true, 0, KS>),
                          hipFuncAttributeMaxDynamicSharedMemorySize, (int)lds);
      (void)hipFuncSetAttribute(reinterpret_cast<const void*>(
                              conv3x3_mfma_kernel<WM, WN, NT, false, 0, KS>),
                          hipFuncAttributeMaxDynamicSharedMemorySize, (int)lds);
      attr_set = true;
    }
  }
  long long blocks = (long long)a.tiles_x * a.tiles_y * a.nocg * n * a.ksplit;
  TG_REQUIRE(blocks > 0 && blocks < (1ll << 31), TG_E_SHAPE, "conv3x3: grid %lld", blocks);
  static const int xcd_env = TG_LAB_ENV("TG_CONV_XCD", -1);
  const bool xcd = xcd_env >= 0 ? xcd_env != 0 : blocks >= 512;
  a.nblocks = xcd ? (int)blocks : 0;
  const unsigned grid = xcd ? (unsigned)(8 * ((blocks + 7) / 8)) : (unsigned)blocks;
  if (a.x2)
    hipLaunchKernelGGL((conv3x3_mfma_kernel<WM, WN, NT, true, 0, KS>),
                       dim3(grid), dim3(WM * WN * KS * 64), lds, stream, a);
  else
    hipLaunchKernelGGL((conv3x3_mfma_kernel<WM, WN, NT, false, 0, KS>),
                       dim3(grid), dim3(WM * WN * KS * 64), lds, stream, a);
  return check_launch("conv3x3_mfma");
}

__global__ void splitk_finalize_kernel(const float* __restrict__ part, int S, long long part_ss,
                                       const float* __restrict__ bias, float slope, int pool,
                                       float* __restrict__ y, int n, int c, int h, int w) {
  const int oh = pool ? h / 2 : h, ow = pool ? w / 2 : w;
  const long long total = (long long)n * c * oh * ow;
  for (long long i = (long long)blockIdx.x * blockDim.x + threadIdx.x; i < total;
       i += (long long)gridDim.x * blockDim.x) {
    int ox = (int)(i % ow); long long t = i / ow;
    int oy = (int)(t % oh); t /= oh;
    int ch = (int)(t % c);
    long long plane = t * h * (long long)w;
    float b = bias ? bias[ch] : 0.f;
    auto at = [&](int yy, int xx) {
      const float* p = part + plane + (long long)yy * w + xx;
      float v = 0.f;
      for (int s = 0; s < S; ++s) v += p[(long long)s * part_ss];
      v += b;
      return v >= 0.f ? v : v * slope + 0.f;
    };
    float v;
    if (pool) {
      v = fmaxf(fmaxf(at(2 * oy, 2 * ox), at(2 * oy, 2 * ox + 1)),
                fmaxf(at(2 * oy + 1, 2 * ox), at(2 * oy + 1, 2 * ox + 1)));
    } else {
      v = at(oy, ox);
    }
    y[i] = v;
  }
}

}

namespace tg {
bool conv3x3_uses_oneshot(int n, int cin, int cout, int h, int w) {
  static const int env = TG_LAB_ENV("TG_CONV_ONESHOT", 1);
  return env && cout <= 64 && cdiv(cin, CK) <= 8 && conv3x3_uses_wg_ksplit(n, cin, cout, h, w);
}

bool conv3x3_uses_wg_ksplit(int n, int cin, int cout, int h, int w) {
  static const int ks_env = TG_LAB_ENV("TG_CONV_WG_KSPLIT", 1);
  if (!ks_env || tg_conv3x3_pick_ocb(cout) != 64 || conv3x3_rows_per_wg(64, (long long)n * h * w) != 2)
    return false;
  const long long wgs2 = (long long)cdiv(w, TW) * cdiv(h, 2) * cdiv(cout, 64) * n;
  return wgs2 <= 128 && cdiv(cin, CK) >= 6;
}
}

using namespace tg;

extern "C" int tg_conv3x3_pick_ksplit(int n, int cin, int cout, int h, int w) {
  int ocb = tg_conv3x3_pick_ocb(cout);
  int rows = conv3x3_rows_per_wg(ocb, (long long)n * h * w);
  const double wgs = (double)cdiv(w, TW) * cdiv(h, rows) * cdiv(cout, ocb) * n;
  const int nchunk = cdiv(cin, CK);
  if (conv3x3_uses_oneshot(n, cin, cout, h, w)) return 1;
  static const int legacy = TG_LAB_ENV("TG_KSPLIT_LEGACY", 0);
  if (legacy) {
    if (wgs >= 400 || nchunk < 4) return 1;
    int ks = 1;
    while (ks < 8 && wgs * ks < 640 && nchunk / (ks * 2) >= 2) ks *= 2;
    return ks;
  }
  auto cost = [&](int ks) {
    double share = wgs * ks / 256.0;
    return 4.0 + 1.15 * ((double)nchunk / ks) * (share > 1.0 ? share : 1.0) + (ks > 1 ? 4.5 : 0.0);
  };
  int best = 1;
  double tbest = cost(1);
  for (int ks = 2; ks <= 8 && nchunk / ks >= 2; ks *= 2) {
    double t = cost(ks);
    if (t < 0.85 * tbest) { best = ks; tbest = t; }
  }
  return best;
}

extern "C" int tg_conv3x3_pick_ocb(int cout) { return cout <= 32 ? 32 : 64; }

extern "C" size_t tg_conv3x3_packed_floats(int cin, int cout, int ocb) {
  if (cin <= 0 || cout <= 0 || (ocb != 32 && ocb != 64)) return 0;
  return (size_t)cdiv(cout, ocb) * cdiv(cin, CK) * 9 * CK * ocb;
}

extern "C" int tg_conv3x3_pack(const float* w, float* w_packed, int cin, int cout,
                               int ocb, int transposed, tg_stream_t stream) {
  TG_REQUIRE(w && w_packed, TG_E_ARG, "conv3x3_pack: null pointer");
  TG_REQUIRE(cin > 0 && cout > 0 && (ocb == 32 || ocb == 64), TG_E_SHAPE,
             "conv3x3_pack: cin=%d cout=%d ocb=%d", cin, cout, ocb);
  int nchunk = cdiv(cin, CK), nocg = cdiv(cout, ocb);
  int total = nocg * nchunk * 9 * CK * ocb;
  int blocks = cdiv(total, 256);
  if (blocks > 4096) blocks = 4096;
  hipLaunchKernelGGL(pack3x3_kernel, dim3(blocks), dim3(256), 0, (hipStream_t)stream, w,
                     w_packed, cin, cout, ocb, nchunk, nocg, transposed);
  return check_launch("pack3x3");
}

static int conv3x3_impl(const float* x, int64_t x_nstride, int c1, const float* x2,
                        int64_t x2_nstride, const float* w_packed, int ocb, const float* bias,
                        const float* res, int64_t res_nstride, float* y, int64_t y_nstride, int n,
                        int cin, int cout, int h, int w, int act, int ksplit, float* partials,
                        tg_stream_t stream, const float* mask = nullptr, int64_t mask_nstride = 0,
                        int tapsel = 0, int cphase = 0, int set_p0 = 0, int set_p1 = 0) {
  TG_REQUIRE(x && w_packed && y, TG_E_ARG, "conv3x3_fwd: null pointer");
  TG_REQUIRE(!mask || ksplit <= 1, TG_E_ARG, "conv3x3_fwd: the ReLU mask is applied in the epilogue (no split-K)");
  TG_REQUIRE(n > 0 && cin > 0 && cout > 0 && h > 0 && w > 0, TG_E_SHAPE,
             "conv3x3_fwd: n=%d cin=%d cout=%d h=%d w=%d", n, cin, cout, h, w);
  TG_REQUIRE(c1 > 0 && c1 <= cin && (c1 == cin || x2), TG_E_ARG,
             "conv3x3_fwd: c1=%d cin=%d needs a second source", c1, cin);
  TG_REQUIRE(act >= TG_ACT_NONE && act <= TG_ACT_LRELU02, TG_E_ARG,
             "conv3x3_fwd: act=%d (none|relu|lrelu; tanh*24 only in tg_conv3x3_small_fwd)", act);
  TG_REQUIRE(ocb == 32 || ocb == 64, TG_E_ARG, "conv3x3_fwd: ocb=%d", ocb);
  TG_REQUIRE((long long)(cin + CK) * h * w * 4 < (1ll << 31), TG_E_SHAPE,
             "conv3x3_fwd: one batch item must be < 2 GiB (cin=%d h=%d w=%d)", cin, h, w);
  Conv3x3Args a{};
  a.x = x; a.x2 = (c1 < cin) ? x2 : nullptr; a.wpk = w_packed; a.bias = bias; a.res = res;
  a.y = y; a.x_ns = x_nstride; a.x2_ns = x2_nstride; a.res_ns = res_nstride; a.y_ns = y_nstride;
  a.c1 = c1; a.cin = cin; a.cout = cout; a.h = h; a.w = w; a.act = act;
  a.ksplit = ksplit; a.part = partials; a.part_ss = (long long)n * cout * h * w;
  a.mask = mask; a.mask_ns = mask_nstride;
  a.tapsel = tapsel; a.cphase = cphase; a.rowsets[0] = (unsigned char)set_p0; a.rowsets[1] = (unsigned char)set_p1;
  if (tapsel) {
    TG_REQUIRE((tapsel == 1 || tapsel == 2) && cphase > 0 && cphase % CK == 0 && set_p0 >= 0 && set_p0 <= 3 &&
                   set_p1 >= 0 && set_p1 <= 3, TG_E_ARG, "conv3x3: tapsel=%d cphase=%d sets %d/%d", tapsel,
               cphase, set_p0, set_p1);
    TG_REQUIRE(tapsel == 1 ? cin == 4 * cphase : (cout == 4 * cphase && cphase % 64 == 0), TG_E_SHAPE,
               "conv3x3: phased taps need 4 phases of %d channels (cin=%d cout=%d)", cphase, cin, cout);
  }
  hipStream_t s = (hipStream_t)stream;
  if (ocb == 32) return launch_conv<4, 1, 1>(a, n, s);
  if (conv3x3_rows_per_wg(ocb, (long long)n * h * w) == 4) return launch_conv<4, 1, 2>(a, n, s);
  if (a.ksplit <= 1 && !tapsel && conv3x3_uses_oneshot(n, cin, cout, h, w)) {
    a.vec_ok = (a.w % 4 == 0) && ((uintptr_t)a.y % 16 == 0) && (a.y_ns % 4 == 0) &&
               (!a.res || (((uintptr_t)a.res % 16 == 0) && (a.res_ns % 4 == 0))) &&
               (!a.mask || (((uintptr_t)a.mask % 16 == 0) && (a.mask_ns % 4 == 0)));
    a.tiles_x = cdiv(a.w, TW); a.tiles_y = a.h; a.nocg = 1; a.nchunk = cdiv(a.cin, CK);
    const size_t lds = (size_t)(8 * 3 * 2 * RS * 4 + 2 * 3 * 16 * 64) * sizeof(float);
    static bool attr_set = false;
    if (!attr_set) {
      (void)hipFuncSetAttribute(reinterpret_cast<const void*>(conv3x3_oneshot_kernel<true>),
                                hipFuncAttributeMaxDynamicSharedMemorySize, (int)lds);
      (void)hipFuncSetAttribute(reinterpret_cast<const void*>(conv3x3_oneshot_kernel<false>),
                                hipFuncAttributeMaxDynamicSharedMemorySize, (int)lds);
      attr_set = true;
    }
    const unsigned grid = (unsigned)(a.tiles_x * a.tiles_y * n);
    if (a.x2) hipLaunchKernelGGL(conv3x3_oneshot_kernel<true>, dim3(grid), dim3(512), lds, s, a);
    else hipLaunchKernelGGL(conv3x3_oneshot_kernel<false>, dim3(grid), dim3(512), lds, s, a);
    return check_launch("conv3x3_oneshot");
  }
  if (a.ksplit <= 1 && conv3x3_uses_wg_ksplit(n, cin, cout, h, w)) return launch_conv<1, 2, 1, 2>(a, n, s);
  return launch_conv<2, 2, 1>(a, n, s);
}

extern "C" int tg_conv3x3_fwd(const float* x, int64_t x_nstride, int c1, const float* x2,
                              int64_t x2_nstride, const float* w_packed, int ocb,
                              const float* bias, const float* res, int64_t res_nstride,
                              float* y, int64_t y_nstride, int n, int cin, int cout, int h,
                              int w, int act, tg_stream_t stream) {
  return conv3x3_impl(x, x_nstride, c1, x2, x2_nstride, w_packed, ocb, bias, res, res_nstride, y,
                      y_nstride, n, cin, cout, h, w, act, 1, nullptr, stream);
}

extern "C" int tg_conv3x3_fwd_phased(const float* x, int64_t x_nstride, const float* w_packed, int ocb,
                                     const float* bias, float* y, int64_t y_nstride, int n, int cin,
                                     int cout, int h, int w, int act, int tapsel, int cphase,
                                     int taps_phase0, int taps_phase1, tg_stream_t stream) {
  TG_REQUIRE(tapsel == 1 || tapsel == 2, TG_E_ARG, "conv3x3_fwd_phased: tapsel=%d (1 input | 2 output phases)", tapsel);
  return conv3x3_impl(x, x_nstride, cin, nullptr, 0, w_packed, ocb, bias, nullptr, 0, y, y_nstride, n, cin,
                      cout, h, w, act, 1, nullptr, stream, nullptr, 0, tapsel, cphase, taps_phase0,
                      taps_phase1);
}

extern "C" int tg_conv3x3_fwd_phased_masked(const float* x, int64_t x_nstride, const float* w_packed, int ocb,
                                            const float* bias, const float* relu_mask, int64_t mask_nstride,
                                            float* y, int64_t y_nstride, int n, int cin, int cout, int h,
                                            int w, int act, int tapsel, int cphase, int taps_phase0,
                                            int taps_phase1, tg_stream_t stream) {
  TG_REQUIRE(tapsel == 1 || tapsel == 2, TG_E_ARG, "conv3x3_fwd_phased: tapsel=%d (1 input | 2 output phases)", tapsel);
  return conv3x3_impl(x, x_nstride, cin, nullptr, 0, w_packed, ocb, bias, nullptr, 0, y, y_nstride, n, cin,
                      cout, h, w, act, 1, nullptr, stream, relu_mask, mask_nstride, tapsel, cphase, taps_phase0,
                      taps_phase1);
}

extern "C" int tg_conv3x3_phased_pick_ksplit(int n, int cin, int cout, int h, int w, int ocb) {
  if (n <= 0 || cin <= 0 || cout <= 0 || h <= 0 || w <= 0 || (ocb != 32 && ocb != 64)) return 1;
  const int rows = conv3x3_rows_per_wg(ocb, (long long)n * h * w);
  const long long wgs = (long long)cdiv(w, TW) * cdiv(h, rows) * cdiv(cout, ocb) * n;
  const int nchunk = cdiv(cin, CK);
  if (wgs >= 384 || nchunk < 16) return 1;
  int ks = 2;
  while (ks < 8 && wgs * ks * 2 <= 1024 && nchunk / (ks * 2) >= 4) ks *= 2;
  return ks;
}

extern "C" int tg_conv3x3_fwd_phased_splitk(const float* x, int64_t x_nstride, const float* w_packed, int ocb,
                                            const float* bias, float* y, int n, int cin, int cout, int h, int w,
                                            int act, int tapsel, int cphase, int taps_phase0, int taps_phase1,
                                            int ksplit, float* partials, tg_stream_t stream) {
  TG_REQUIRE(y && partials, TG_E_ARG, "conv3x3_fwd_phased_splitk: null pointer");
  TG_REQUIRE(tapsel == 1 || tapsel == 2, TG_E_ARG, "conv3x3_fwd_phased_splitk: tapsel=%d", tapsel);
  TG_REQUIRE(ksplit >= 2 && ksplit <= 16 && ksplit <= cdiv(cin, CK), TG_E_ARG,
             "conv3x3_fwd_phased_splitk: ksplit=%d for cin=%d", ksplit, cin);
  TG_REQUIRE(act >= TG_ACT_NONE && act <= TG_ACT_LRELU02, TG_E_ARG, "conv3x3_fwd_phased_splitk: act=%d", act);
  int rc = conv3x3_impl(x, x_nstride, cin, nullptr, 0, w_packed, ocb, nullptr, nullptr, 0, partials,
                        (int64_t)cout * h * w, n, cin, cout, h, w, TG_ACT_NONE, ksplit, partials, stream, nullptr, 0,
                        tapsel, cphase, taps_phase0, taps_phase1);
  if (rc != TG_OK) return rc;
  return conv3x3_splitk_finalize(partials, ksplit, bias, act, 0, y, n, cout, h, w, stream);
}

static const int S2_MAX_TILES = 1024;
extern "C" int tg_conv3x3s2_supported(int n, int cin, int cout, int h_out, int w_out) {
  if (n <= 0 || cin <= 0 || cin > 64 || cout <= 0 || cout > 64 || h_out <= 0 || w_out <= 0) return 0;
  return (long long)n * h_out * cdiv(w_out, TW) <= S2_MAX_TILES ? 1 : 0;
}

extern "C" int tg_conv3x3s2_fwd(const float* x, int64_t x_nstride, const float* w_packed, const float* bias,
                                const float* relu_mask, int64_t mask_nstride, float* y, int64_t y_nstride, int n,
                                int cin, int cout, int h_out, int w_out, int act, tg_stream_t stream) {
  TG_REQUIRE(x && w_packed && y, TG_E_ARG, "conv3x3s2_fwd: null pointer");
  TG_REQUIRE(tg_conv3x3s2_supported(n, cin, cout, h_out, w_out), TG_E_SHAPE,
             "conv3x3s2_fwd: n=%d cin=%d cout=%d out %dx%d (cin, cout <= 64, <= 1024 row tiles)", n, cin, cout, h_out, w_out);
  TG_REQUIRE(act >= TG_ACT_NONE && act <= TG_ACT_LRELU02, TG_E_ARG, "conv3x3s2_fwd: act=%d", act);
  TG_REQUIRE((long long)(cin + CK) * 4 * h_out * w_out * 4 < (1ll << 31), TG_E_SHAPE, "conv3x3s2_fwd: item too large");
  Conv3x3Args a{};
  a.x = x; a.wpk = w_packed; a.bias = bias; a.y = y; a.x_ns = x_nstride; a.y_ns = y_nstride;
  a.mask = relu_mask; a.mask_ns = mask_nstride;
  a.c1 = cin; a.cin = cin; a.cout = cout; a.h = h_out; a.w = w_out; a.act = act;
  a.tiles_x = cdiv(w_out, TW); a.tiles_y = h_out; a.nocg = 1; a.nchunk = cdiv(cin, CK);
  const size_t lds = (size_t)(8 * 3 * 2 * RS2 * 4 + 2 * 3 * 16 * 64) * sizeof(float);
  static bool attr_set = false;
  if (!attr_set) {
    (void)hipFuncSetAttribute(reinterpret_cast<const void*>(conv3x3s2_oneshot_kernel),
                              hipFuncAttributeMaxDynamicSharedMemorySize, (int)lds);
    attr_set = true;
  }
  hipLaunchKernelGGL(conv3x3s2_oneshot_kernel, dim3((unsigned)(a.tiles_x * a.tiles_y * n)), dim3(512), lds,
                     (hipStream_t)stream, a);
  return check_launch("conv3x3s2_oneshot");
}

extern "C" int tg_conv3x3_fwd_masked(const float* x, int64_t x_nstride, int c1, const float* x2,
                                     int64_t x2_nstride, const float* w_packed, int ocb,
// ... 44 lines not shown
```

### tecogan-pytorch_amd/csrc/tg_conv3x3_wino.hip

```cpp
#include <stdlib.h>

#include "tg_common.h"

namespace tg {

struct WinoArgs {
  const float* x;
  const float* x2;
  const float* u;
  const float* bias;
  const float* res;
  const float* mask;
  float* y;
  long long x_ns, x2_ns, res_ns, mask_ns, y_ns;
  int c1, cin, cout, h, w, act;
  int tiles_x, tiles_y, nstage, nocg, nocb;
  int nblocks;
  int vec_ok;
};

constexpr int W_ICS = 16;
constexpr int W_RS = 40;
constexpr int W_ICSTR = 4 * W_RS;
constexpr int W_VS = 20;

__global__ void wino_pack_kernel(const float* __restrict__ w, float* __restrict__ out, int cin, int cout,
                                 int nchunk, int nocb, int transposed) {
  const int total = nchunk * nocb * 4 * 64 * 4;
  for (int i = blockIdx.x * blockDim.x + threadIdx.x; i < total; i += gridDim.x * blockDim.x) {
    const int e = i & 3, lane = (i >> 2) & 63, j = (i >> 8) & 3;
    const int rest = i >> 10;
    const int ocb = rest % nocb, chunk = rest / nocb;
    const int p = 4 * j + e;
    const int oc = 16 * ocb + (lane & 15), ic = 4 * chunk + (lane >> 4);
    float v = 0.f;
    if (oc < cout && ic < cin) {
      float g[3][3];
#pragma unroll
      for (int a = 0; a < 3; ++a)
#pragma unroll
        for (int b = 0; b < 3; ++b)
          g[a][b] = transposed == 2 ? w[((size_t)ic * cout + oc) * 9 + (8 - (a * 3 + b))]
                                    : w[((size_t)oc * cin + ic) * 9 + a * 3 + b];
      const int pi = p >> 2, pj = p & 3;
      float col[3];
#pragma unroll
      for (int b = 0; b < 3; ++b) {
        col[b] = pi == 0 ? g[0][b]
               : pi == 1 ? 0.5f * ((g[0][b] + g[1][b]) + g[2][b])
               : pi == 2 ? 0.5f * ((g[0][b] - g[1][b]) + g[2][b])
                         : g[2][b];
      }
      v = pj == 0 ? col[0]
        : pj == 1 ? 0.5f * ((col[0] + col[1]) + col[2])
        : pj == 2 ? 0.5f * ((col[0] - col[1]) + col[2])
                  : col[2];
    }
    out[i] = v;
  }
}

template <bool COH> __device__ __forceinline__ float2 ld2(const float* p) {
  if constexpr (COH) {
    const unsigned long long v = __hip_atomic_load(reinterpret_cast<const unsigned long long*>(p), __ATOMIC_RELAXED, __HIP_MEMORY_SCOPE_AGENT);
    return make_float2(__builtin_bit_cast(float, (unsigned)v), __builtin_bit_cast(float, (unsigned)(v >> 32)));
  } else {
    return *reinterpret_cast<const float2*>(p);
  }
}
template <bool COH> __device__ __forceinline__ float ld1(const float* p) {
  if constexpr (COH) return __hip_atomic_load(p, __ATOMIC_RELAXED, __HIP_MEMORY_SCOPE_AGENT);
  else return *p;
}
template <bool COH> __device__ __forceinline__ void st2(float* p, float v0, float v1) {
  if constexpr (COH) {
    const unsigned long long v = (unsigned long long)__builtin_bit_cast(unsigned, v0) | ((unsigned long long)__builtin_bit_cast(unsigned, v1) << 32);
    __hip_atomic_store(reinterpret_cast<unsigned long long*>(p), v, __ATOMIC_RELAXED, __HIP_MEMORY_SCOPE_AGENT);
  } else {
    *reinterpret_cast<float2*>(p) = make_float2(v0, v1);
  }
}
template <bool COH> __device__ __forceinline__ void st1(float* p, float v) {
  if constexpr (COH) __hip_atomic_store(p, v, __ATOMIC_RELAXED, __HIP_MEMORY_SCOPE_AGENT);
  else *p = v;
}

constexpr int AUX_SC1 = 16;

template <int TR> struct WGeo3 {
  static constexpr int TC = 16 / TR;
  static constexpr int PR = 2 * TR + 2, PC = 2 * TC + 2;
  static constexpr int PE = PR * PC;
  static constexpr int RS = TR == 1 ? W_RS : (TR == 2 ? 24 : 12);
  static_assert(PR * RS <= W_ICSTR, "patch of one channel fits the channel stride");
};

template <bool COH, int TR = 1>
__device__ __forceinline__ void wino_tile(const WinoArgs& a, int tx, int ty, int ocg, int n) {
  using G = WGeo3<TR>;
  __shared__ __attribute__((aligned(16))) float s_raw[W_ICS * W_ICSTR];
  __shared__ __attribute__((aligned(16))) float s_v[2 * W_ICS * 16 * W_VS];

  const int t = threadIdx.x, l = t & 63;
  const int wv = __builtin_amdgcn_readfirstlane(t >> 6);
  const int x0 = tx * (2 * G::TC), y0 = ty * (2 * TR);
  const int hw = a.h * a.w;

  constexpr int RAW_ELEMS = W_ICS * G::PE;
  constexpr int RAW_PER_T = (RAW_ELEMS + 255) / 256;
  constexpr unsigned OOB = 0x80000000u;
  unsigned roff[RAW_PER_T];
#pragma unroll
  for (int k = 0; k < RAW_PER_T; ++k) {
    const int e = t + 256 * k;
    const int ic = e / G::PE, rem = e - ic * G::PE, r = rem / G::PC, c = rem - r * G::PC;
    const int gy = y0 - 1 + r, gx = x0 - 1 + c;
    roff[k] = (e < RAW_ELEMS && gy >= 0 && gy < a.h && gx >= 0 && gx < a.w)
                  ? (unsigned)(ic * hw + gy * a.w + gx) * 4u : OOB;
  }
  const __amdgpu_buffer_rsrc_t rx = __builtin_amdgcn_make_buffer_rsrc(
      const_cast<float*>(a.x + (size_t)n * a.x_ns), 0, (unsigned)a.c1 * hw * 4u, 0x00020000);
  const __amdgpu_buffer_rsrc_t rx2 = __builtin_amdgcn_make_buffer_rsrc(
      const_cast<float*>(a.x2 ? a.x2 + (size_t)n * a.x2_ns : a.x), 0,
      a.x2 ? (unsigned)(a.cin - a.c1) * hw * 4u : 0u, 0x00020000);
  const bool dual = a.x2 != nullptr;
  auto load_raw = [&](int s, float (&reg)[RAW_PER_T]) {
    const unsigned so = (unsigned)(s * W_ICS) * hw * 4u;
#pragma unroll
    for (int k = 0; k < RAW_PER_T; ++k) {
      float v = __builtin_bit_cast(float, __builtin_amdgcn_raw_buffer_load_b32(rx, (int)(roff[k] + so), 0, COH ? AUX_SC1 : 0));
      if (dual)
        v += __builtin_bit_cast(float, __builtin_amdgcn_raw_buffer_load_b32(
                 rx2, (int)(roff[k] + so - (unsigned)a.c1 * hw * 4u), 0, COH ? AUX_SC1 : 0));
      reg[k] = v;
    }
  };
  auto store_raw = [&](const float (&reg)[RAW_PER_T]) {
#pragma unroll
    for (int k = 0; k < RAW_PER_T; ++k) {
      const int e = t + 256 * k;
      const int ic = e / G::PE, rem = e - ic * G::PE, r = rem / G::PC, c = rem - r * G::PC;
      if (e < RAW_ELEMS) s_raw[ic * W_ICSTR + r * G::RS + c] = reg[k];
    }
  };

  const f32x4* ug = reinterpret_cast<const f32x4*>(a.u) + ((size_t)(ocg * 4 + wv) * 4) * 64 + l;
  const size_t ustep = (size_t)a.nocb * 4 * 64;
  const int ktotal = 4 * a.nstage;
  auto load_uh = [&](int kstep, int half, f32x4 (&u)[4]) {
    kstep = kstep < ktotal ? kstep : ktotal - 1;
    const f32x4* p = ug + (size_t)kstep * ustep + half * 128;
    u[2 * half] = p[0];
    u[2 * half + 1] = p[64];
  };

  f32x4 acc[16];
#pragma unroll
  for (int p = 0; p < 16; ++p) acc[p] = f32x4{0.f, 0.f, 0.f, 0.f};

  constexpr int VBUF4 = W_ICS * 16 * W_VS / 4;
  const float* traw = s_raw + (t >> 4) * W_ICSTR + 2 * ((t & 15) / G::TC) * G::RS + 2 * ((t & 15) % G::TC);
  f32x4* tv = reinterpret_cast<f32x4*>(s_v + t * W_VS);
  const f32x4* bv = reinterpret_cast<const f32x4*>(s_v + ((l >> 4) * 16 + (l & 15)) * W_VS);

  auto mfma8 = [&](const f32x4 (&u)[4], int buf, int ks, int half) {
    f32x4 bq[2];
#pragma unroll
    for (int j = 0; j < 2; ++j) bq[j] = bv[buf * VBUF4 + ks * (4 * 16 * W_VS / 4) + 2 * half + j];
#pragma unroll
    for (int p = 0; p < 8; ++p)
      acc[8 * half + p] = __builtin_amdgcn_mfma_f32_16x16x4f32(u[2 * half + (p >> 2)][p & 3], bq[p >> 2][p & 3],
                                                               acc[8 * half + p], 0, 0, 0);
  };
  auto kstep = [&](int k, f32x4 (&u)[4], int buf, auto&& between) {
    mfma8(u, buf, k & 3, 0);
    __builtin_amdgcn_sched_barrier(0);
    load_uh(k + 2, 0, u);
    between();
    mfma8(u, buf, k & 3, 1);
    __builtin_amdgcn_sched_barrier(0);
    load_uh(k + 2, 1, u);
  };
  auto transform_half = [&](int buf, int hp) {
    float d[3][4];
#pragma unroll
    for (int r = 0; r < 3; ++r) {
      const float2 p0 = *reinterpret_cast<const float2*>(traw + (r + hp) * G::RS);
      const float2 p1 = *reinterpret_cast<const float2*>(traw + (r + hp) * G::RS + 2);
      d[r][0] = p0.x; d[r][1] = p0.y; d[r][2] = p1.x; d[r][3] = p1.y;
    }
    float qa[4], qb[4];
#pragma unroll
    for (int c = 0; c < 4; ++c) {
      qa[c] = hp == 0 ? d[0][c] - d[2][c] : d[1][c] - d[0][c];
      qb[c] = hp == 0 ? d[1][c] + d[2][c] : d[0][c] - d[2][c];
    }
    tv[buf * VBUF4 + 2 * hp] = f32x4{qa[0] - qa[2], qa[1] + qa[2], qa[2] - qa[1], qa[1] - qa[3]};
    tv[buf * VBUF4 + 2 * hp + 1] = f32x4{qb[0] - qb[2], qb[1] + qb[2], qb[2] - qb[1], qb[1] - qb[3]};
  };

  const int ox = x0 + 2 * ((l & 15) % G::TC);
  const int oy0 = y0 + 2 * ((l & 15) / G::TC);
  const int oc_base = ocg * 64 + wv * 16 + 4 * (l >> 4);
  const float* rn = a.res ? a.res + (size_t)n * a.res_ns : nullptr;
  const bool res_pre = rn && a.vec_ok;

  float rawreg[RAW_PER_T];
  f32x4 u0[4], u1[4];
  const int last = a.nstage - 1;
  load_raw(0, rawreg);
  load_uh(0, 0, u0); load_uh(0, 1, u0);
  load_uh(1, 0, u1); load_uh(1, 1, u1);
  store_raw(rawreg);
  __syncthreads();
  if (last > 0) load_raw(1, rawreg);
  transform_half(0, 0);
  transform_half(0, 1);
  __syncthreads();
  if (last > 0) store_raw(rawreg);

  auto nothing = [] {};
  for (int s = 0; s < last; ++s) {
    const int cur = s & 1, nxt = cur ^ 1;
    kstep(4 * s + 0, u0, cur, nothing);
    __syncthreads();
    if (s + 2 <= last) load_raw(s + 2, rawreg);
    kstep(4 * s + 1, u1, cur, [&] { transform_half(nxt, 0); });
    kstep(4 * s + 2, u0, cur, [&] { transform_half(nxt, 1); });
    kstep(4 * s + 3, u1, cur, nothing);
    __syncthreads();
    if (s + 2 <= last) store_raw(rawreg);
  }
  float2 rpre[4][2];
  {
    const int cur = last & 1;
    kstep(4 * last + 0, u0, cur, nothing);
    kstep(4 * last + 1, u1, cur, nothing);
    kstep(4 * last + 2, u0, cur, nothing);
#pragma unroll
    for (int r = 0; r < 4; ++r)
#pragma unroll
      for (int i = 0; i < 2; ++i) {
        rpre[r][i] = make_float2(0.f, 0.f);
        if (res_pre && oc_base + r < a.cout && ox < a.w && oy0 + i < a.h)
          rpre[r][i] = ld2<COH>(rn + (size_t)(oc_base + r) * hw + (size_t)(oy0 + i) * a.w + ox);
      }
    kstep(4 * last + 3, u1, cur, nothing);
  }

  const float slope = act_slope(a.act);
  float* yn = a.y + (size_t)n * a.y_ns;
  const float* mn = a.mask ? a.mask + (size_t)n * a.mask_ns : nullptr;
#pragma unroll
  for (int r = 0; r < 4; ++r) {
    const int oc = oc_base + r;
    float sr[2][4];
#pragma unroll
    for (int j = 0; j < 4; ++j) {
      sr[0][j] = (acc[0 + j][r] + acc[4 + j][r]) + acc[8 + j][r];
      sr[1][j] = (acc[4 + j][r] - acc[8 + j][r]) - acc[12 + j][r];
    }
    if (oc >= a.cout || ox >= a.w) continue;
    const float bz = a.bias ? a.bias[oc] : 0.f;
#pragma unroll
    for (int i = 0; i < 2; ++i) {
      const int oy = oy0 + i;
      if (oy >= a.h) continue;
      float v0 = ((sr[i][0] + sr[i][1]) + sr[i][2]) + bz;
      float v1 = ((sr[i][1] - sr[i][2]) - sr[i][3]) + bz;
      if (a.act == TG_ACT_TANH24) { v0 = apply_act(v0, a.act); v1 = apply_act(v1, a.act); }
      else {
        v0 = __builtin_fmaxf(v0, slope * v0);
        v1 = __builtin_fmaxf(v1, slope * v1);
      }
      const size_t o = (size_t)oc * hw + (size_t)oy * a.w + ox;
      const bool two = ox + 1 < a.w;
      if (a.vec_ok) {
        if (rn) { v0 += rpre[r][i].x; v1 += rpre[r][i].y; }
        if (mn) { const float2 mm = *reinterpret_cast<const float2*>(mn + o); v0 = mm.x > 0.f ? v0 : 0.f; v1 = mm.y > 0.f ? v1 : 0.f; }
        st2<COH>(yn + o, v0, v1);
      } else {
        if (rn) { v0 += ld1<COH>(rn + o); if (two) v1 += ld1<COH>(rn + o + 1); }
        if (mn) { v0 = mn[o] > 0.f ? v0 : 0.f; if (two) v1 = mn[o + 1] > 0.f ? v1 : 0.f; }
        st1<COH>(yn + o, v0);
        if (two) st1<COH>(yn + o + 1, v1);
      }
    }
  }
}

template <int TR>
__global__ __launch_bounds__(256, 3) void conv3x3_wino_kernel(WinoArgs a) {
  int b = blockIdx.x;
  if (a.nblocks > 0) {
    const int per = (a.nblocks + 7) >> 3;
    b = (b & 7) * per + (b >> 3);
    if (b >= a.nblocks) return;
  }
  const int tx = __builtin_amdgcn_readfirstlane(b % a.tiles_x); b /= a.tiles_x;
  const int ty = __builtin_amdgcn_readfirstlane(b % a.tiles_y); b /= a.tiles_y;
  const int ocg = __builtin_amdgcn_readfirstlane(b % a.nocg);
  const int n = __builtin_amdgcn_readfirstlane(b / a.nocg);
  wino_tile<false, TR>(a, tx, ty, ocg, n);
}

struct WinoLayer {
  const float *x, *x2, *u, *bias, *res;
  float* y;
  long long x_ns, x2_ns, res_ns, y_ns;
  int c1, cin, act, nstage;
};
constexpr int W_MAX_CHAIN = 24;
struct WinoChainArgs {
  WinoLayer L[W_MAX_CHAIN];
  int nlayer, bpl;
  int cout, h, w, tiles_x, tiles_y, ntile, vec_ok;
  int* flags;
  int* err;
  unsigned epoch;
  int poll_limit;
};

template <bool COHX>
__global__ __launch_bounds__(256, 3) void conv3x3_wino_chain_kernel(WinoChainArgs c) {
  const int layer = __builtin_amdgcn_readfirstlane((int)blockIdx.x / c.bpl);
  int b = (int)blockIdx.x - layer * c.bpl;
  {
    const int per = c.bpl >> 3;
    b = (b & 7) * per + (b >> 3);
    if (b >= c.ntile) return;
  }
  const int tile = b;
  const int tx = __builtin_amdgcn_readfirstlane(b % c.tiles_x); b /= c.tiles_x;
  const int ty = __builtin_amdgcn_readfirstlane(b % c.tiles_y);
  const int n = __builtin_amdgcn_readfirstlane(b / c.tiles_y);
  const WinoLayer& L = c.L[layer];
  WinoArgs a;
  a.x = L.x; a.x2 = L.x2; a.u = L.u; a.bias = L.bias; a.res = L.res; a.mask = nullptr; a.y = L.y;
  a.x_ns = L.x_ns; a.x2_ns = L.x2_ns; a.res_ns = L.res_ns; a.mask_ns = 0; a.y_ns = L.y_ns;
  a.c1 = L.c1; a.cin = L.cin; a.cout = c.cout; a.h = c.h; a.w = c.w; a.act = L.act;
  a.tiles_x = c.tiles_x; a.tiles_y = c.tiles_y; a.nstage = L.nstage; a.nocg = 1; a.nocb = 4;
  a.nblocks = 0; a.vec_ok = c.vec_ok;
  if (layer > 0) {
    const int t = threadIdx.x;
    if (t < 9) {
      const int ny = ty - 1 + t / 3, nx = tx - 1 + t % 3;
      if (ny >= 0 && ny < c.tiles_y && nx >= 0 && nx < c.tiles_x) {
        const unsigned* f = reinterpret_cast<const unsigned*>(c.flags) + (size_t)(layer - 1) * c.ntile + (n * c.tiles_y + ny) * c.tiles_x + nx;
        int polls = 0;
        bool fault = c.poll_limit < 0;
        while (!fault && __hip_atomic_load(f, __ATOMIC_RELAXED, __HIP_MEMORY_SCOPE_AGENT) != c.epoch) {
          __builtin_amdgcn_s_sleep(4);
          fault = ++polls > c.poll_limit;
        }
        if (fault) __hip_atomic_fetch_add(c.err, 1, __ATOMIC_RELAXED, __HIP_MEMORY_SCOPE_SYSTEM);
      }
    }
    __syncthreads();
  }
  wino_tile<COHX>(a, tx, ty, 0, n);
  __builtin_amdgcn_s_waitcnt(0);
  __syncthreads();
  if (threadIdx.x == 0)
    __hip_atomic_store(reinterpret_cast<unsigned*>(c.flags) + (size_t)layer * c.ntile + tile, c.epoch, __ATOMIC_RELAXED, __HIP_MEMORY_SCOPE_AGENT);
}

}

using namespace tg;

extern "C" int64_t tg_conv3x3_wino_packed_floats(int cin, int cout) {
  if (cin <= 0 || cout <= 0) return -1;
  const int64_t nchunk = 4 * ((cin + 15) / 16), nocb = 4 * ((cout + 63) / 64);
  return nchunk * nocb * 4 * 64 * 4;
}

extern "C" int tg_conv3x3_prefers_wino(int n, int cin, int cout, int h, int w) {
  static const int env = [] { const char* e = getenv("TG_CONV_WINO"); return e && *e ? atoi(e) : -1; }();
  if (env == 0) return 0;
  if (n <= 0 || cin < 16 || cout <= 0 || cout % 64 != 0 || h < 2 || w < 2) return 0;
  const long long wgs = (long long)cdiv(w, 32) * cdiv(h, 2) * (cout / 64) * n;
  return env == 1 ? 1 : (wgs >= 160 ? 1 : 0);
}

extern "C" int tg_pack_conv3x3_wino(const float* w, float* out, int cin, int cout, int transposed,
                                    tg_stream_t stream) {
  TG_REQUIRE(w && out, TG_E_ARG, "pack_conv3x3_wino: null pointer");
  TG_REQUIRE(cin > 0 && cout > 0 && (transposed == 0 || transposed == 2), TG_E_ARG,
             "pack_conv3x3_wino: cin=%d cout=%d transposed=%d (0 or 2)", cin, cout, transposed);
  const int nchunk = 4 * cdiv(cin, 16), nocb = 4 * cdiv(cout, 64);
  const int total = nchunk * nocb * 4 * 64 * 4;
  hipLaunchKernelGGL(wino_pack_kernel, dim3(cdiv(total, 256) > 1024 ? 1024 : cdiv(total, 256)), dim3(256), 0,
                     (hipStream_t)stream, w, out, cin, cout, nchunk, nocb, transposed);
  return check_launch("pack_conv3x3_wino");
}

namespace tg {
int conv3x3_wino_launch(const float* x, int64_t x_ns, int c1, const float* x2, int64_t x2_ns, const float* u,
                        const float* bias, const float* res, int64_t res_ns, const float* mask,
                        int64_t mask_ns, float* y, int64_t y_ns, int n, int cin, int cout, int h, int w,
                        int act, tg_stream_t stream) {
  WinoArgs a{};
  a.x = x; a.x2 = x2; a.u = u; a.bias = bias; a.res = res; a.mask = mask; a.y = y;
  a.x_ns = x_ns; a.x2_ns = x2_ns; a.res_ns = res_ns; a.mask_ns = mask_ns; a.y_ns = y_ns;
  a.c1 = x2 ? c1 : cin; a.cin = cin; a.cout = cout; a.h = h; a.w = w; a.act = act;
  int tr = 1;
  {
    long long best = (long long)cdiv(w, 32) * cdiv(h, 2);
    for (int cand = 2; cand <= 4; cand *= 2) {
      const long long c = (long long)cdiv(w, 32 / cand) * cdiv(h, 2 * cand);
      if (c < best) { best = c; tr = cand; }
    }
    static const int tr_env = TG_LAB_ENV("TG_WINO_TR", 0);
    if (tr_env == 1 || tr_env == 2 || tr_env == 4) tr = tr_env;
  }
  a.tiles_x = cdiv(w, 32 / tr); a.tiles_y = cdiv(h, 2 * tr);
  a.nstage = cdiv(cin, 16); a.nocg = cdiv(cout, 64); a.nocb = 4 * a.nocg;
  auto al8 = [](const void* p, int64_t ns) { return ((uintptr_t)p % 8) == 0 && ns % 2 == 0; };
  a.vec_ok = (w % 2 == 0) && ((int64_t)h * w) % 2 == 0 && al8(y, y_ns) && (!res || al8(res, res_ns)) &&
             (!mask || al8(mask, mask_ns));
  const long long blocks = (long long)a.tiles_x * a.tiles_y * a.nocg * n;
  static const int xcd_env = TG_LAB_ENV("TG_WINO_XCD", -1);
  const bool xcd = xcd_env >= 0 ? xcd_env != 0 : blocks >= 512;
  a.nblocks = xcd ? (int)blocks : 0;
  const unsigned grid = xcd ? (unsigned)(8 * ((blocks + 7) / 8)) : (unsigned)blocks;
  if (tr == 1) hipLaunchKernelGGL(conv3x3_wino_kernel<1>, dim3(grid), dim3(256), 0, (hipStream_t)stream, a);
  else if (tr == 2) hipLaunchKernelGGL(conv3x3_wino_kernel<2>, dim3(grid), dim3(256), 0, (hipStream_t)stream, a);
  else hipLaunchKernelGGL(conv3x3_wino_kernel<4>, dim3(grid), dim3(256), 0, (hipStream_t)stream, a);
  return check_launch("conv3x3_wino");
}
}

extern "C" int tg_conv3x3_wino_fwd(const float* x, int64_t x_nstride, int c1, const float* x2,
                                   int64_t x2_nstride, const float* u_packed, const float* bias,
                                   const float* res, int64_t res_nstride, const float* relu_mask,
                                   int64_t mask_nstride, float* y, int64_t y_nstride, int n, int cin,
                                   int cout, int h, int w, int act, tg_stream_t stream) {
  TG_REQUIRE(x && u_packed && y, TG_E_ARG, "conv3x3_wino: null pointer");
  TG_REQUIRE(n > 0 && cin > 0 && cout > 0 && h > 0 && w > 0, TG_E_SHAPE, "conv3x3_wino: n=%d cin=%d cout=%d h=%d w=%d",
             n, cin, cout, h, w);
  TG_REQUIRE(!x2 || (c1 > 0 && c1 < cin), TG_E_ARG, "conv3x3_wino: c1=%d of cin=%d", c1, cin);
  TG_REQUIRE(act >= TG_ACT_NONE && act <= TG_ACT_TANH24, TG_E_ARG, "conv3x3_wino: act=%d", act);
  TG_REQUIRE((long long)cin * h * w < (1ll << 29), TG_E_SHAPE, "conv3x3_wino: image too large");
  return conv3x3_wino_launch(x, x_nstride, c1, x2, x2_nstride, u_packed, bias, res, res_nstride, relu_mask,
                             mask_nstride, y, y_nstride, n, cin, cout, h, w, act, stream);
}

extern "C" int64_t tg_conv3x3_wino_chain_flag_ints(int n_layers, int n, int h, int w) {
  if (n_layers <= 0 || n_layers > W_MAX_CHAIN || n <= 0 || h <= 0 || w <= 0) return -1;
  return (int64_t)n_layers * n * cdiv(h, 2) * cdiv(w, 32) + 16;
}

namespace tg {
int conv3x3_wino_chain_launch(const tg_wino_layer* layers, int n_layers, int n, int cout, int h, int w,
                              int32_t* flags, int32_t* err, unsigned epoch, int poll_limit, tg_stream_t stream) {
  TG_REQUIRE(layers && flags && err, TG_E_ARG, "conv3x3_wino_chain: null pointer");
  TG_REQUIRE(n_layers >= 1 && n_layers <= W_MAX_CHAIN, TG_E_ARG, "conv3x3_wino_chain: %d layers (1..%d)", n_layers, W_MAX_CHAIN);
  TG_REQUIRE(n > 0 && h > 0 && w > 0 && cout > 0 && cout <= 64, TG_E_SHAPE,
             "conv3x3_wino_chain: n=%d cout=%d (<= 64: one output-channel group) h=%d w=%d", n, cout, h, w);
  TG_REQUIRE(epoch != 0, TG_E_ARG, "conv3x3_wino_chain: epoch 0 is the cleared state of the flags");
  WinoChainArgs c{};
  c.nlayer = n_layers; c.cout = cout; c.h = h; c.w = w;
  c.tiles_x = cdiv(w, 32); c.tiles_y = cdiv(h, 2);
  const long long ntile = (long long)c.tiles_x * c.tiles_y * n;
  TG_REQUIRE(ntile * n_layers < (1ll << 30), TG_E_SHAPE, "conv3x3_wino_chain: too many tiles");
  c.ntile = (int)ntile;
  c.bpl = (int)(8 * ((ntile + 7) / 8));
  c.flags = flags; c.err = err; c.epoch = epoch; c.poll_limit = poll_limit;
  bool vec = (w % 2 == 0) && ((int64_t)h * w) % 2 == 0;
  auto al8 = [](const void* p, int64_t ns) { return ((uintptr_t)p % 8) == 0 && ns % 2 == 0; };
  for (int i = 0; i < n_layers; ++i) {
    const tg_wino_layer& l = layers[i];
    TG_REQUIRE(l.x && l.u_packed && l.y, TG_E_ARG, "conv3x3_wino_chain: layer %d: null pointer", i);
    TG_REQUIRE(l.cin > 0 && (!l.x2 || (l.c1 > 0 && l.c1 < l.cin)), TG_E_ARG, "conv3x3_wino_chain: layer %d: cin=%d c1=%d", i, l.cin, l.c1);
    TG_REQUIRE((long long)l.cin * h * w < (1ll << 29), TG_E_SHAPE, "conv3x3_wino_chain: layer %d too large", i);
    TG_REQUIRE(l.act >= TG_ACT_NONE && l.act <= TG_ACT_TANH24, TG_E_ARG, "conv3x3_wino_chain: layer %d: act=%d", i, l.act);
    WinoLayer& d = c.L[i];
    d.x = l.x; d.x2 = l.x2; d.u = l.u_packed; d.bias = l.bias; d.res = l.res; d.y = l.y;
    d.x_ns = l.x_nstride; d.x2_ns = l.x2_nstride; d.res_ns = l.res_nstride; d.y_ns = l.y_nstride;
    d.c1 = l.x2 ? l.c1 : l.cin; d.cin = l.cin; d.act = l.act; d.nstage = cdiv(l.cin, 16);
    vec = vec && al8(l.y, l.y_nstride) && (!l.res || al8(l.res, l.res_nstride));
  }
  c.vec_ok = vec ? 1 : 0;
  const unsigned grid = (unsigned)(c.bpl * n_layers);
#if TG_LAB
  static const int noncoh = TG_LAB_ENV("TG_WINO_CHAIN_NONCOH", 0);
  static const int pad_lds = TG_LAB_ENV("TG_WINO_CHAIN_LDS", 0);
  if (noncoh) {
    hipLaunchKernelGGL(conv3x3_wino_chain_kernel<false>, dim3(grid), dim3(256), pad_lds, (hipStream_t)stream, c);
    return check_launch("conv3x3_wino_chain");
  }
  hipLaunchKernelGGL(conv3x3_wino_chain_kernel<true>, dim3(grid), dim3(256), pad_lds, (hipStream_t)stream, c);
#else
  hipLaunchKernelGGL(conv3x3_wino_chain_kernel<true>, dim3(grid), dim3(256), 0, (hipStream_t)stream, c);
#endif
  return check_launch("conv3x3_wino_chain");
}
}

extern "C" int tg_conv3x3_wino_chain(const tg_wino_layer* layers, int n_layers, int n, int cout, int h, int w,
                                     int32_t* flags, int epoch, tg_stream_t stream) {
  TG_REQUIRE(flags && n_layers >= 1 && n > 0 && h > 0 && w > 0, TG_E_ARG, "conv3x3_wino_chain: bad argument");
  const long long ntile = (long long)cdiv(w, 32) * cdiv(h, 2) * n;
  return conv3x3_wino_chain_launch(layers, n_layers, n, cout, h, w, flags, flags + (size_t)n_layers * ntile,
                                   (unsigned)epoch, TG_CHAIN_POLL_LIMIT_DEFAULT, stream);
}
```

### tecogan-pytorch_amd/ops.py

```python
import torch

from . import _lib as L
from ._lib import (ACT_NONE, ACT_RELU, ACT_LRELU02, ACT_TANH24,
                   UP_NONE, UP_BICUBIC, UP_BILINEAR)

UP_MODE = {'BD': UP_BICUBIC, 'BI': UP_BILINEAR}


_RAW_STREAM = getattr(torch._C, '_cuda_getCurrentRawStream', None)


def _stream():
    if _RAW_STREAM is not None:
        return _RAW_STREAM(torch.cuda.current_device())
    return torch.cuda.current_stream().cuda_stream


def _chk(t, name, dtype=torch.float32):
    if not (torch.is_tensor(t) and t.is_cuda):
        raise L.TecoganHipError(f'{name}: expected a CUDA/HIP tensor (no CPU path exists)')
    if t.dtype != dtype:
        raise L.TecoganHipError(f'{name}: expected {dtype}, got {t.dtype}')
    if not t.is_contiguous():
        raise L.TecoganHipError(f'{name}: tensor must be contiguous')
    return t


def _ptr(t):
    return None if t is None else t.data_ptr()


def param_version(w):
    return (w.data_ptr(), w._version, getattr(w, '_tg_version', 0))


def bump_version(w):
    w._tg_version = getattr(w, '_tg_version', 0) + 1


def pick_ocb(cout):
    return L.lib().tg_conv3x3_pick_ocb(int(cout))


def pack_conv3x3(weight, transposed=False, ocb=None):
    w = _chk(weight.detach(), 'weight')
    if w.dim() != 4 or w.shape[2:] != (3, 3):
        raise L.TecoganHipError(f'pack_conv3x3: weight shape {tuple(w.shape)}')
    if transposed:
        cin, cout = w.shape[0], w.shape[1]
        ocb = 64
    else:
        cout, cin = w.shape[0], w.shape[1]
        ocb = ocb or pick_ocb(cout)
    nfl = L.lib().tg_conv3x3_packed_floats(cin, cout, ocb)
    out = torch.empty(nfl, dtype=torch.float32, device=w.device)
    L.check(L.lib().tg_conv3x3_pack(w.data_ptr(), out.data_ptr(), cin, cout, ocb,
                                    1 if transposed else 0, _stream()), 'tg_conv3x3_pack')
    return out, cin, cout, ocb


def conv3x3(x, wpk, bias, cin, cout, ocb, act=ACT_NONE, x2=None, res=None, out=None,
            pool=False, ksplit=None, relu_mask=None):
    _chk(x, 'x')
    n, c1, h, w = x.shape
    if ksplit is None:
        ksplit = 1 if (res is not None or relu_mask is not None) else \
            L.lib().tg_conv3x3_pick_ksplit(n, cin, cout, h, w)
    if ksplit > 1:
        if res is not None or relu_mask is not None:
            raise L.TecoganHipError('conv3x3: split-K path has no residual / mask epilogue')
        if x2 is not None:
            _chk(x2, 'x2')
        part = torch.empty(ksplit * n * cout * h * w, dtype=torch.float32, device=x.device)
        oh, ow = (h // 2, w // 2) if pool else (h, w)
        if out is None:
            out = torch.empty(n, cout, oh, ow, dtype=torch.float32, device=x.device)
        L.check(L.lib().tg_conv3x3_splitk_fwd(
            x.data_ptr(), c1 * h * w, c1, _ptr(x2), 0 if x2 is None else x2.shape[1] * h * w,
            wpk.data_ptr(), ocb, _ptr(bias), out.data_ptr(), n, cin, cout, h, w, act, ksplit,
            part.data_ptr(), 1 if pool else 0, _stream()), 'tg_conv3x3_splitk_fwd')
        return out
    if pool:
        return maxpool2(conv3x3(x, wpk, bias, cin, cout, ocb, act, x2=x2, res=res, ksplit=1))
    if x2 is not None:
        _chk(x2, 'x2')
        if x2.shape[0] != n or x2.shape[2:] != x.shape[2:] or c1 + x2.shape[1] != cin:
            raise L.TecoganHipError(f'conv3x3: x {tuple(x.shape)} x2 {tuple(x2.shape)} cin {cin}')
    elif c1 != cin:
        raise L.TecoganHipError(f'conv3x3: x has {c1} channels, weights expect {cin}')
    if out is None:
        out = torch.empty(n, cout, h, w, dtype=torch.float32, device=x.device)
    _chk(out, 'out')
    if res is not None:
        _chk(res, 'res')
        if res.shape != out.shape:
            raise L.TecoganHipError('conv3x3: residual shape mismatch')
    hw = h * w
    if relu_mask is not None:
        _chk(relu_mask, 'relu_mask')
        if relu_mask.shape != out.shape:
            raise L.TecoganHipError('conv3x3: relu_mask shape mismatch')
        L.check(L.lib().tg_conv3x3_fwd_masked(
            x.data_ptr(), c1 * hw, c1, _ptr(x2), 0 if x2 is None else x2.shape[1] * hw,
            wpk.data_ptr(), ocb, _ptr(bias), _ptr(res), cout * hw, relu_mask.data_ptr(), cout * hw,
            out.data_ptr(), cout * hw, n, cin, cout, h, w, act, _stream()), 'tg_conv3x3_fwd_masked')
        return out
    L.check(L.lib().tg_conv3x3_fwd(
        x.data_ptr(), c1 * hw, c1, _ptr(x2), 0 if x2 is None else x2.shape[1] * hw,
        wpk.data_ptr(), ocb, _ptr(bias), _ptr(res), cout * hw, out.data_ptr(), cout * hw,
        n, cin, cout, h, w, act, _stream()), 'tg_conv3x3_fwd')
    return out


TAPS_ALL, TAPS_01, TAPS_12, TAPS_1 = 0, 1, 2, 3


def conv3x3_phased(x, wpk, cin, cout, ocb, tapsel, cphase, taps_phase0, taps_phase1, out=None, relu_mask=None):
    _chk(x, 'x')
    n, c1, h, w = x.shape
    if c1 != cin:
        raise L.TecoganHipError(f'conv3x3_phased: x has {c1} channels, weights expect {cin}')
    if out is None:
        out = torch.empty(n, cout, h, w, dtype=torch.float32, device=x.device)
    if relu_mask is not None:
        _chk(relu_mask, 'relu_mask')
        if relu_mask.shape != out.shape:
            raise L.TecoganHipError('conv3x3_phased: relu_mask shape mismatch')
    ks = 1 if relu_mask is not None or not out.is_contiguous() else \
        L.lib().tg_conv3x3_phased_pick_ksplit(n, cin, cout, h, w, ocb)
    if ks > 1:
        part = torch.empty(ks * n * cout * h * w, dtype=torch.float32, device=x.device)
        L.check(L.lib().tg_conv3x3_fwd_phased_splitk(x.data_ptr(), cin * h * w, wpk.data_ptr(), ocb, None,
                                                     out.data_ptr(), n, cin, cout, h, w, ACT_NONE, int(tapsel),
                                                     int(cphase), int(taps_phase0), int(taps_phase1), ks,
                                                     part.data_ptr(), _stream()), 'tg_conv3x3_fwd_phased_splitk')
        return out
    L.check(L.lib().tg_conv3x3_fwd_phased_masked(x.data_ptr(), cin * h * w, wpk.data_ptr(), ocb, None,
                                                 _ptr(relu_mask), cout * h * w, out.data_ptr(), cout * h * w,
                                                 n, cin, cout, h, w, ACT_NONE, int(tapsel), int(cphase),
                                                 int(taps_phase0), int(taps_phase1), _stream()),
            'tg_conv3x3_fwd_phased_masked')
    return out


def pack_conv3x3_m16(weight, transposed=0):
    w = _chk(weight.detach().contiguous(), 'weight')
    cout, cin = w.shape[0], w.shape[1]
    out = torch.empty(L.lib().tg_conv3x3_pack16_floats(), dtype=torch.float32, device=w.device)
    if transposed == 2:
        L.check(L.lib().tg_conv3x3_pack16(w.data_ptr(), out.data_ptr(), cout, cin, 2, _stream()), 'tg_conv3x3_pack16')
    else:
        L.check(L.lib().tg_conv3x3_pack16(w.data_ptr(), out.data_ptr(), cin, cout, 0, _stream()), 'tg_conv3x3_pack16')
    return out


def chain_pack(items, layout):
    lib = L.lib()
    arr = (L.PackItem * len(items))()
    sizes = []
    for wt, i_off, i_cnt, tr in items:
        _chk(wt, 'weight')
        cin, cout = (wt.shape[0], i_cnt) if tr == 2 else (i_cnt, wt.shape[0])
        sizes.append(int(lib.tg_conv3x3_chain_packed_floats(layout, cin)))
    buf = torch.empty(sum(sizes), dtype=torch.float32, device=items[0][0].device)
    outs, off = [], 0
    for a, (wt, i_off, i_cnt, tr), sz in zip(arr, items, sizes):
        o = buf[off:off + sz]; off += sz
        outs.append(o)
        a.w, a.out, a.transposed, a.i_total, a.i_off = wt.data_ptr(), o.data_ptr(), tr, wt.shape[1], i_off
        a.cin, a.cout = (wt.shape[0], i_cnt) if tr == 2 else (i_cnt, wt.shape[0])
    L.check(lib.tg_conv3x3_chain_pack(arr, len(items), layout, _stream()), 'tg_conv3x3_chain_pack')
    return outs


def conv3x3s2_supported(n, cin, cout, h_out, w_out):
    return bool(L.lib().tg_conv3x3s2_supported(n, cin, cout, h_out, w_out))


def conv3x3s2(x, wpk, cin, cout, relu_mask=None, out=None):
    _chk(x, 'x')
    n, c, h2, w2 = x.shape
    if c != cin or h2 % 2 or w2 % 2:
        raise L.TecoganHipError(f'conv3x3s2: x {tuple(x.shape)} cin {cin}')
    h, w = h2 // 2, w2 // 2
    if out is None:
        out = torch.empty(n, cout, h, w, dtype=torch.float32, device=x.device)
    elif tuple(out.shape) != (n, cout, h, w):
        raise L.TecoganHipError(f'conv3x3s2: out {tuple(out.shape)}')
    else:
        _chk(out, 'out')
    if relu_mask is not None:
        _chk(relu_mask, 'relu_mask')
        if relu_mask.shape != out.shape:
# ... 887 lines not shown
            'tg_time_gather')
    return out


def pingpong(x):
    t = x.shape[1]
    return time_gather(x, list(range(t)) + list(range(t - 2, -1, -1)))


def pingpong_grad(g, te):
    _chk(g, 'g')
    n = g.shape[0]
    inner = g[0, 0].numel()
    out = torch.empty((n, 2 * te - 1) + tuple(g.shape[2:]), dtype=torch.float32, device=g.device)
    L.check(L.lib().tg_pingpong_grad(g.data_ptr(), out.data_ptr(), n, te, inner, _stream()), 'tg_pingpong_grad')
    return out


def d_assemble_fwd(data, warped, cond, t, pad, crop, out=None):
    _chk(data, 'data'); _chk(warped, 'warped'); _chk(cond, 'cond')
    n, t_data, c, h, w = data.shape
    x = out if out is not None else torch.empty(n * t // 3, 9 * c, h, w, dtype=torch.float32, device=data.device)
    L.check(L.lib().tg_d_assemble_fwd(data.data_ptr(), t_data, warped.data_ptr(), cond.data_ptr(),
                                      cond.shape[1], x.data_ptr(), n, t, c, h, w, pad, crop, _stream()),
            'tg_d_assemble_fwd')
    return x


def d_assemble_bwd(g, n, t, t_data, c, pad, crop):
    _chk(g, 'g')
    h, w = g.shape[2:]
    g_data = torch.empty(n, t_data, c, h, w, dtype=torch.float32, device=g.device)
    g_warped = torch.empty(n * t, c, h, w, dtype=torch.float32, device=g.device)
    L.check(L.lib().tg_d_assemble_bwd(g.data_ptr(), g_data.data_ptr(), t_data, g_warped.data_ptr(), n, t, c,
                                      h, w, pad, crop, _stream()), 'tg_d_assemble_bwd')
    return g_data, g_warped


def transpose01(x):
    _chk(x, 'x')
    a, b = x.shape[:2]
    y = torch.empty((b, a) + tuple(x.shape[2:]), dtype=torch.float32, device=x.device)
    L.check(L.lib().tg_transpose01(x.data_ptr(), y.data_ptr(), a, b, x[0, 0].numel(), _stream()),
            'tg_transpose01')
    return y


def stack_time(frames):
    import ctypes
    for f in frames:
        _chk(f, 'frame')
    n = frames[0].shape[0]
    y = torch.empty((n, len(frames)) + tuple(frames[0].shape[1:]), dtype=torch.float32,
                    device=frames[0].device)
    arr = (ctypes.c_void_p * len(frames))(*[f.data_ptr() for f in frames])
    L.check(L.lib().tg_stack_time(arr, len(frames), y.data_ptr(), n, frames[0][0].numel(), _stream()),
            'tg_stack_time')
    return y


def index_gather(src, idx, out=None, accumulate=False):
    _chk(src, 'src'); _chk(idx, 'idx', torch.int64)
    if out is None:
        assert not accumulate
        out = torch.empty(idx.numel(), dtype=torch.float32, device=src.device)
    else:
        _chk(out, 'out')
        assert out.numel() == idx.numel()
    L.check(L.lib().tg_index_gather(src.data_ptr(), idx.data_ptr(), out.data_ptr(), idx.numel(),
                                    src.numel(), int(accumulate), _stream()), 'tg_index_gather')
    return out


def pack_conv3x3_wino(w, transposed=0):
    _chk(w, 'w')
    co, ci = (w.shape[0], w.shape[1]) if transposed == 0 else (w.shape[1], w.shape[0])
    nflt = L.lib().tg_conv3x3_wino_packed_floats(ci, co)
    out = torch.empty(nflt, dtype=torch.float32, device=w.device)
    L.check(L.lib().tg_pack_conv3x3_wino(w.data_ptr(), out.data_ptr(), ci, co, transposed, _stream()),
            'tg_pack_conv3x3_wino')
    return out


def conv3x3_wino(x, u_packed, bias, cin, cout, act=ACT_NONE, x2=None, res=None, mask=None, out=None):
    _chk(x, 'x'); _chk(u_packed, 'u_packed')
    n, c1, h, w = x.shape
    if x2 is not None:
        _chk(x2, 'x2')
        assert c1 + x2.shape[1] == cin
    else:
        assert c1 == cin
    y = out if out is not None else torch.empty(n, cout, h, w, dtype=torch.float32, device=x.device)
    L.check(L.lib().tg_conv3x3_wino_fwd(
        x.data_ptr(), x.stride(0), c1, _ptr(x2), x2.stride(0) if x2 is not None else 0,
        u_packed.data_ptr(), _ptr(bias), _ptr(res), res.stride(0) if res is not None else 0,
        _ptr(mask), mask.stride(0) if mask is not None else 0, y.data_ptr(), y.stride(0),
        n, cin, cout, h, w, act, _stream()), 'tg_conv3x3_wino_fwd')
    return y


class RowChain:

    def __init__(self, layers, n, h, w):
        lib = L.lib()
        self.n, self.h, self.w = n, h, w
        self.parts = lib.tg_conv3x3_chain_supported(n, h, w, 64)
        if self.parts == 0:
            raise L.TecoganHipError(f'RowChain: {n}x{h}x{w} cannot run as a chained launch on this device')
        self.layout = 16 if self.parts == 4 else 64
        self.keep = [layers]
        self.arr = (L.ChainLayer * len(layers))()
        for i, d in enumerate(layers):
            a = self.arr[i]
            wt = d['w']
            pk = pack_conv3x3_m16(wt) if self.layout == 16 else pack_conv3x3(wt, ocb=64)[0]
            self.keep.append(pk)
            x, x2, res, mask, y = d['x'], d.get('x2'), d.get('res'), d.get('mask'), d['y']
            a.x, a.x2, a.w_packed, a.bias = x.data_ptr(), _ptr(x2), pk.data_ptr(), _ptr(d.get('bias'))
            a.res, a.relu_mask, a.y = _ptr(res), _ptr(mask), y.data_ptr()
            a.x_nstride, a.y_nstride = x.stride(0), y.stride(0)
            a.x2_nstride = x2.stride(0) if x2 is not None else 0
            a.res_nstride = res.stride(0) if res is not None else 0
            a.mask_nstride = mask.stride(0) if mask is not None else 0
            a.c1, a.cin, a.cout, a.act = x.shape[1], wt.shape[1], wt.shape[0], d.get('act', ACT_NONE)
        self.nl = len(layers)
        self.flags = torch.zeros(lib.tg_conv3x3_chain_flag_ints(self.nl, n, h, w) + 16, dtype=torch.int32,
                                 device=layers[0]['x'].device)
        self.err = self.flags[-16:]
        self.epoch = 0

    def run(self, poll_limit=1 << 21):
        self.epoch += 1
        L.check(L.lib().tg_conv3x3_chain(self.arr, self.nl, self.n, self.h, self.w, self.layout, self.flags.data_ptr(),
                                         self.err.data_ptr(), self.epoch, poll_limit, _stream()), 'tg_conv3x3_chain')

    def faults(self):
        return int(self.err[0].item())


class WinoChain:

    def __init__(self, layers, n, cout, h, w):
        import ctypes
        self.n, self.cout, self.h, self.w = n, cout, h, w
        self.keep = layers
        self.arr = (L.WinoLayer * len(layers))()
        for i, d in enumerate(layers):
            a = self.arr[i]
            x, x2, res, y = d['x'], d.get('x2'), d.get('res'), d['y']
            a.x, a.x2, a.u_packed = x.data_ptr(), _ptr(x2), d['u'].data_ptr()
            a.bias, a.res, a.y = _ptr(d.get('bias')), _ptr(res), y.data_ptr()
            a.x_nstride, a.y_nstride = x.stride(0), y.stride(0)
            a.x2_nstride = x2.stride(0) if x2 is not None else 0
            a.res_nstride = res.stride(0) if res is not None else 0
            a.c1, a.cin, a.act = x.shape[1], d['cin'], d.get('act', ACT_NONE)
        nints = L.lib().tg_conv3x3_wino_chain_flag_ints(len(layers), n, h, w)
        self.flags = torch.zeros(nints, dtype=torch.int32, device=layers[0]['x'].device)
        self.epoch = 0

    def run(self):
        self.epoch += 1
        L.check(L.lib().tg_conv3x3_wino_chain(self.arr, len(self.keep), self.n, self.cout, self.h, self.w,
                                              self.flags.data_ptr(), self.epoch, _stream()),
                'tg_conv3x3_wino_chain')

    def bailouts(self):
        return int(self.flags[-16].item())


def pack_wres_convt(w):
    _chk(w, 'w')
    if tuple(w.shape) != (64, 64, 3, 3):
        raise L.TecoganHipError(f'pack_wres_convt: weight {tuple(w.shape)}, expected (64, 64, 3, 3)')
    lib = L.lib()
# ... 105 lines not shown
```

Baseline: 1536 frames/s.

## Fold maxpool into conv epilogue and bilinear upsample into conv input staging

Adds a glue variant of the 32-channel MFMA conv kernel. It can max-pool 2x2 in its epilogue, or build a 2x bilinear upsample of its input on the fly while staging tiles to LDS. It also adds a pooled-epilogue Winograd kernel. The FNet encoder/decoder then skips the separate pool and upsample launches and their full-resolution intermediate writes and reads. In exchange the conv does extra interpolation math per staged tile, uses a fixed 4x1 tile shape, and adds branching in the host-side scheduling.

New measurement: 1545 frames/s, median of 6. No clear change (+0.6%).

```diff
diff --git a/include/tecogan_hip.h b/include/tecogan_hip.h
--- a/include/tecogan_hip.h
+++ b/include/tecogan_hip.h
@@ -47,6 +47,11 @@
     const float* res, int64_t res_nstride,
     float* y, int64_t y_nstride,
     int n, int cin, int cout, int h, int w, int act, tg_stream_t stream);
+
+int tg_conv3x3_glue_supported(int n, int cin, int cout, int h, int w, int ocb, int pool, int up2);
+int tg_conv3x3_glue_fwd(const float* x, int64_t x_nstride, int c1, const float* x2, int64_t x2_nstride,
+                        const float* w_packed, int ocb, const float* bias, float* y, int64_t y_nstride,
+                        int n, int cin, int cout, int h, int w, int act, int pool, int up2, tg_stream_t stream);
 
 int tg_conv3x3_fwd_phased(const float* x, int64_t x_nstride, const float* w_packed, int ocb,
                           const float* bias, float* y, int64_t y_nstride, int n, int cin,
@@ -90,6 +95,11 @@
                         const float* res, int64_t res_nstride, const float* relu_mask,
                         int64_t mask_nstride, float* y, int64_t y_nstride, int n, int cin,
                         int cout, int h, int w, int act, tg_stream_t stream);
+
+int tg_conv3x3_wino_pool_supported(int h, int w);
+int tg_conv3x3_wino_pool_fwd(const float* x, int64_t x_nstride, int c1, const float* x2, int64_t x2_nstride,
+                             const float* u_packed, const float* bias, float* y, int64_t y_nstride, int n,
+                             int cin, int cout, int h, int w, int act, tg_stream_t stream);
 
 typedef struct {
   const float* x; const float* x2; const float* u_packed; const float* bias; const float* res;
diff --git a/tecogan-pytorch_amd/_lib.py b/tecogan-pytorch_amd/_lib.py
--- a/tecogan-pytorch_amd/_lib.py
+++ b/tecogan-pytorch_amd/_lib.py
@@ -169,6 +169,10 @@
     'tg_conv3x3_prefers_wino': (I, [I, I, I, I, I]),
     'tg_pack_conv3x3_wino': (I, [P, P, I, I, I, P]),
     'tg_conv3x3_wino_fwd': (I, [P, I64, I, P, I64, P, P, P, I64, P, I64, P, I64, I, I, I, I, I, I, P]),
+    'tg_conv3x3_wino_pool_supported': (I, [I, I]),
+    'tg_conv3x3_wino_pool_fwd': (I, [P, I64, I, P, I64, P, P, P, I64, I, I, I, I, I, I, P]),
+    'tg_conv3x3_glue_supported': (I, [I, I, I, I, I, I, I, I]),
+    'tg_conv3x3_glue_fwd': (I, [P, I64, I, P, I64, P, I, P, P, I64, I, I, I, I, I, I, I, I, P]),
     'tg_time_gather': (I, [P, P, P, I, I, I, I64, P]),
     'tg_transpose01': (I, [P, P, I, I, I64, P]),
     'tg_stack_time': (I, [P, I, P, I, I64, P]),
diff --git a/tecogan-pytorch_amd/csrc/tg_api.hip b/tecogan-pytorch_amd/csrc/tg_api.hip
--- a/tecogan-pytorch_amd/csrc/tg_api.hip
+++ b/tecogan-pytorch_amd/csrc/tg_api.hip
@@ -249,7 +249,8 @@
   K_F16_PACK = 17,
   K_F16_CONV = 18,
   K_F16_CONVT = 19,
-  K_COUNT = 20
+  K_CONV32_GLUE = 20,
+  K_COUNT = 21
 };
 
 static bool hr_fuse_enabled() {
@@ -295,9 +296,19 @@
     }
     if (active && (mask & (1u << kind))) rc = fn();
   };
+  auto up2_folds = [&](const tg_layer_weights& lw, int cin, int cout, int hh, int ww) {
+    if (lw.u && tg_conv3x3_prefers_wino(n, cin, cout, hh, ww)) return false;
+    if (tg_conv3x3_pick_ksplit(n, cin, cout, hh, ww) > 1) return false;
+    return tg_conv3x3_glue_supported(n, cin, cout, hh, ww, tg_conv3x3_pick_ocb(cout), 0, 1) != 0;
+  };
+  auto pool_folds = [&](const tg_layer_weights& lw, int cin, int cout, int hh, int ww) {
+    if (lw.u && tg_conv3x3_prefers_wino(n, cin, cout, hh, ww)) return tg_conv3x3_wino_pool_supported(hh, ww) != 0;
+    if (tg_conv3x3_pick_ksplit(n, cin, cout, hh, ww) > 1) return false;
+    return tg_conv3x3_glue_supported(n, cin, cout, hh, ww, tg_conv3x3_pick_ocb(cout), 1, 0) != 0;
+  };
   auto conv = [&](const float* x, int64_t xns, int c1, const float* x2, int64_t x2ns, int cin,
                   int cout, int hh, int ww, int act, const float* res, int64_t rns, float* y,
-                  int64_t yns, bool pool = false, float* pool_tmp = nullptr) {
+                  int64_t yns, bool pool = false, float* pool_tmp = nullptr, bool up2 = false) {
     const tg_layer_weights lw = p->L[li++];
     int ocb = tg_conv3x3_pick_ocb(cout);
     int kind = ocb == 32 ? K_CONV32
@@ -306,7 +317,21 @@
     double px = (double)n * hh * ww;
     double fl = 2.0 * cin * 9 * cout * px;
     double by = 4.0 * px * (cin + cout + (res ? cout : 0)) + 4.0 * 9 * cin * cout;
+    const double by_glue = 4.0 * px * (cin * (up2 ? 0.25 : 1.0) + cout * (pool ? 0.25 : 1.0)) + 4.0 * 9 * cin * cout;
+    if (up2) {
+      go(K_CONV32_GLUE, fl, by_glue, [&] {
+        return tg_conv3x3_glue_fwd(x, xns, c1, nullptr, 0, lw.w, ocb, lw.b, y, yns, n, cin, cout, hh, ww, act, 0, 1, st);
+      });
+      return;
+    }
     if (lw.u && tg_conv3x3_prefers_wino(n, cin, cout, hh, ww)) {
+      if (pool && pool_folds(lw, cin, cout, hh, ww)) {
+        go(K_CONV_WINO, fl, by_glue, [&] {
+          return tg::conv3x3_wino_launch(x, xns, c1, x2, x2ns, lw.u, lw.b, nullptr, 0, nullptr, 0, y, yns, n, cin, cout,
+                                         hh, ww, act, st, true);
+        });
+        return;
+      }
       float* yw = pool ? pool_tmp : y;
       go(K_CONV_WINO, fl, by, [&] {
         return tg::conv3x3_wino_launch(x, xns, c1, x2, x2ns, lw.u, lw.b, res, rns, nullptr, 0, yw,
@@ -328,6 +353,12 @@
       go(K_FINAL, 0, 4.0 * px * cout * (ks + 1), [&] {
         return tg::conv3x3_splitk_finalize(part_buf, ks, lw.b, act, pool ? 1 : 0, y, n, cout, hh, ww,
                                            st);
+      });
+      return;
+    }
+    if (pool && pool_folds(lw, cin, cout, hh, ww)) {
+      go(K_CONV32_GLUE, fl, by_glue, [&] {
+        return tg_conv3x3_glue_fwd(x, xns, c1, x2, x2ns, lw.w, ocb, lw.b, y, yns, n, cin, cout, hh, ww, act, 1, 0, st);
       });
       return;
     }
@@ -352,30 +383,33 @@
     else
       conv(src, (int64_t)cin * hh * ww, cin, nullptr, 0, cin, co, hh, ww, TG_ACT_LRELU02, nullptr,
            0, A, (int64_t)co * hh * ww);
-    conv(A, (int64_t)co * hh * ww, co, nullptr, 0, co, co, hh, ww, TG_ACT_LRELU02, nullptr, 0, A,
+    const bool pf = pool_folds(p->L[li], co, co, hh, ww);
+    conv(A, (int64_t)co * hh * ww, co, nullptr, 0, co, co, hh, ww, TG_ACT_LRELU02, nullptr, 0, pf ? B : A,
          (int64_t)co * (hh / 2) * (ww / 2), true, B);
     hh /= 2; ww /= 2; cin = co;
-    float* t = A; A = B; B = t;
+    if (!pf) { float* t = A; A = B; B = t; }
     src = B;
   }
   const int dec[3] = {256, 128, 64};
+  bool src_up2 = false;
   for (int d = 0; d < 3; ++d) {
     int co = dec[d];
-    conv(src, (int64_t)cin * hh * ww, cin, nullptr, 0, cin, co, hh, ww, TG_ACT_LRELU02, nullptr, 0,
-         A, (int64_t)co * hh * ww);
+    conv(src, (int64_t)cin * (src_up2 ? (hh / 2) * (ww / 2) : hh * ww), cin, nullptr, 0, cin, co, hh, ww, TG_ACT_LRELU02,
+         nullptr, 0, A, (int64_t)co * hh * ww, false, nullptr, src_up2);
     conv(A, (int64_t)co * hh * ww, co, nullptr, 0, co, co, hh, ww, TG_ACT_LRELU02, nullptr, 0, B,
          (int64_t)co * hh * ww);
-    {
+    src_up2 = up2_folds(p->L[li], co, d < 2 ? dec[d + 1] : 32, 2 * hh, 2 * ww);
+    if (!src_up2) {
       float *pi = B, *po = A; int ph = hh, pw = ww;
       go(K_UPSAMPLE, 0, 4.0 * n * co * ph * pw * 5.0,
          [&] { return tg_upsample_fwd(pi, po, n * co, ph, pw, 2, TG_UP_BILINEAR, 1.0f, st); });
+      float* t = A; A = B; B = t;
     }
     hh *= 2; ww *= 2; cin = co;
-    float* t = A; A = B; B = t;
     src = B;
   }
-  conv(src, (int64_t)cin * hh * ww, cin, nullptr, 0, cin, 32, hh, ww, TG_ACT_LRELU02, nullptr, 0, A,
-       (int64_t)32 * hh * ww);
+  conv(src, (int64_t)cin * (src_up2 ? (hh / 2) * (ww / 2) : hh * ww), cin, nullptr, 0, cin, 32, hh, ww, TG_ACT_LRELU02,
+       nullptr, 0, A, (int64_t)32 * hh * ww, false, nullptr, src_up2);
   {
     const tg_layer_weights lw = p->L[li++];
     float* ai = A; int fh_ = hh, fw_ = ww;
@@ -720,7 +754,8 @@
       "splitk_finalize_kernel",      "conv3x3_mfma_kernel<1,2,1,KS=2>",
       "convt3x3s2_mfma_kernel<Z>",   "convout_tail_kernel",        "conv3x3_oneshot_kernel",
       "conv3x3_wino_kernel",         "conv3x3_wino_chain_kernel",  "conv3x3_wino_resident_kernel",
-      "pack_input_f16_kernel",       "conv3x3_f16_kernel<false>",  "conv3x3_f16_kernel<true>"};
+      "pack_input_f16_kernel",       "conv3x3_f16_kernel<false>",  "conv3x3_f16_kernel<true>",
+      "conv3x3_mfma_glue_kernel"};
   return (kind >= 0 && kind < K_COUNT) ? names[kind] : "?";
 }
 
diff --git a/tecogan-pytorch_amd/csrc/tg_common.h b/tecogan-pytorch_amd/csrc/tg_common.h
--- a/tecogan-pytorch_amd/csrc/tg_common.h
+++ b/tecogan-pytorch_amd/csrc/tg_common.h
@@ -59,7 +59,7 @@
 int conv3x3_wino_launch(const float* x, int64_t x_ns, int c1, const float* x2, int64_t x2_ns, const float* u,
                         const float* bias, const float* res, int64_t res_ns, const float* mask,
                         int64_t mask_ns, float* y, int64_t y_ns, int n, int cin, int cout, int h, int w,
-                        int act, tg_stream_t stream);
+                        int act, tg_stream_t stream, bool pool = false);
 
 constexpr int TG_CHAIN_POLL_LIMIT_DEFAULT = 1 << 21;
 int conv3x3_wino_chain_launch(const tg_wino_layer* layers, int n_layers, int n, int cout, int h, int w,
diff --git a/tecogan-pytorch_amd/csrc/tg_conv3x3_mfma.hip b/tecogan-pytorch_amd/csrc/tg_conv3x3_mfma.hip
--- a/tecogan-pytorch_amd/csrc/tg_conv3x3_mfma.hip
+++ b/tecogan-pytorch_amd/csrc/tg_conv3x3_mfma.hip
@@ -106,9 +106,11 @@
   }
 }
 
-template <int WM, int WN, int NT, bool DUAL, int ABL = 0, int KS = 1>
-__global__ __launch_bounds__(WM* WN* KS * 64) void conv3x3_mfma_kernel(Conv3x3Args a) {
+template <int WM, int WN, int NT, bool DUAL, int ABL, int KS, bool POOL, bool UP2>
+__device__ __forceinline__ void conv3x3_mfma_body(const Conv3x3Args& a) {
   static_assert(KS == 1 || KS == 2, "wave groups over K: one or two");
+  static_assert(!POOL || (WM == 4 && WN == 1 && NT == 1 && KS == 1), "pooled epilogue: the 32-channel form");
+  static_assert(!UP2 || !DUAL, "up-sampled input: one source");
   constexpr int NTHREADS = WM * WN * KS * 64;
   constexpr int OCB = WN * NT * 32;
   constexpr int PH = WM + 2;
@@ -142,6 +144,8 @@
   const int n = b / a.ksplit;
   const int x0 = tx * TW, y0 = ty * WM;
   const int hw = a.h * a.w;
+  const int sh = a.h >> 1, sw = a.w >> 1;
+  const int ihw = UP2 ? sh * sw : hw;
   const int ch_begin = (int)((long long)ks * a.nchunk / a.ksplit);
   const int ch_end = (int)((long long)(ks + 1) * a.nchunk / a.ksplit);
 
@@ -154,15 +158,34 @@
     int hf = rem / PW, col = rem - hf * PW;
     int gy = y0 - 1 + r, gx = x0 - 1 + col;
     bool ok = q < IN_ITEMS && gy >= 0 && gy < a.h && gx >= 0 && gx < a.w;
-    voff[i] = ok ? (unsigned)((4 * hf * hw + gy * a.w + gx) * 4) : OOB;
+    voff[i] = ok ? (unsigned)((4 * hf * ihw + (UP2 ? 0 : gy * a.w + gx)) * 4) : OOB;
     lds_item[i] = q < IN_ITEMS ? ((r * 2 + hf) * RS + col) * 4 : -1;
   }
   const __amdgpu_buffer_rsrc_t rs1 = __builtin_amdgcn_make_buffer_rsrc(
-      const_cast<float*>(a.x + (long long)n * a.x_ns), 0, a.c1 * hw * 4, 0x00020000);
+      const_cast<float*>(a.x + (long long)n * a.x_ns), 0, a.c1 * ihw * 4, 0x00020000);
   const __amdgpu_buffer_rsrc_t rs2 = __builtin_amdgcn_make_buffer_rsrc(
       const_cast<float*>(DUAL ? a.x2 + (long long)n * a.x2_ns : a.x), 0,
       DUAL ? (a.cin - a.c1) * hw * 4 : 0, 0x00020000);
-  const unsigned plane = (unsigned)hw * 4u;
+  const unsigned plane = (unsigned)ihw * 4u;
+
+  constexpr int UBC = PW / 2;
+  constexpr int UP_ITEMS = (PH / 2) * UBC * 4;
+  static_assert(!UP2 || (UP_ITEMS <= NTHREADS && PH % 2 == 0 && I_PER_T >= 2 && KS == 1), "one block item per thread");
+  const int u_cp = tid & 1, u_hf = (tid >> 1) & 1, u_br = (tid >> 2) / UBC, u_bc = (tid >> 2) - u_br * UBC;
+  const int u_gy = y0 - 1 + 2 * u_br, u_gx = x0 - 1 + 2 * u_bc;
+  unsigned uoff[4];
+  if constexpr (UP2) {
+    const bool rowA = u_gy >= 0 && u_gy < a.h, rowB = u_gy + 1 < a.h;
+    const bool colA = u_gx >= 0 && u_gx < a.w, colB = u_gx + 1 < a.w;
+    int ys0, ys1, xs0, xs1;
+    float l0, l1;
+    bilinear_src(rowA ? u_gy : u_gy + 1, 2, sh, ys0, ys1, l0, l1);
+    bilinear_src(colA ? u_gx : u_gx + 1, 2, sw, xs0, xs1, l0, l1);
+    const bool on = tid < UP_ITEMS && (rowA || rowB) && (colA || colB);
+    const unsigned ub = on ? (unsigned)((4 * u_hf + 2 * u_cp) * ihw) * 4u : OOB;
+    uoff[0] = ub + (unsigned)(ys0 * sw + xs0) * 4u; uoff[1] = ub + (unsigned)(ys0 * sw + xs1) * 4u;
+    uoff[2] = ub + (unsigned)(ys1 * sw + xs0) * 4u; uoff[3] = ub + (unsigned)(ys1 * sw + xs1) * 4u;
+  }
 
   const f32x4* wsrc =
       reinterpret_cast<const f32x4*>(a.wpk + (size_t)ocg * a.nchunk * W_FLOATS);
@@ -174,6 +197,13 @@
 #pragma unroll
     for (int k = 0; k < KS; ++k) {
       const unsigned cbase = (unsigned)((ch + k) * CK) * plane;
+      if constexpr (UP2) {
+#pragma unroll
+        for (int j = 0; j < 2; ++j)
+#pragma unroll
+          for (int t = 0; t < 4; ++t) rin[k][j][t] = buf_load(rs1, uoff[t] + cbase + (unsigned)j * plane);
+        continue;
+      }
 #pragma unroll
       for (int i = 0; i < I_PER_T; ++i) {
 #pragma unroll
@@ -204,6 +234,35 @@
 #pragma unroll
     for (int k = 0; k < KS; ++k) {
       float* si = s_in + (buf * KS + k) * IN_FLOATS;
+      if constexpr (UP2) {
+        if (tid < UP_ITEMS) {
+#pragma unroll
+          for (int py = 0; py < 2; ++py) {
+            int d0, d1;
+            float ly0, ly1;
+            bilinear_src(u_gy + py, 2, sh, d0, d1, ly0, ly1);
+            const bool oky = u_gy + py >= 0 && u_gy + py < a.h;
+#pragma unroll
+            for (int px = 0; px < 2; ++px) {
+              float lx0, lx1;
+              bilinear_src(u_gx + px, 2, sw, d0, d1, lx0, lx1);
+              const bool ok = oky && u_gx + px >= 0 && u_gx + px < a.w;
+              float o[2];
+#pragma unroll
+              for (int j = 0; j < 2; ++j) {
+                const float ta = rin[k][j][0], tb = rin[k][j][1], ba = rin[k][j][2], bb = rin[k][j][3];
+                float top = lx0 * ta + lx1 * tb;
+                float bot = lx0 * ba + lx1 * bb;
+                float vv = ly0 * top + ly1 * bot;
+                o[j] = ok ? vv : 0.f;
+              }
+              *reinterpret_cast<float2*>(si + (((2 * u_br + py) * 2 + u_hf) * RS + 2 * u_bc + px) * 4 + 2 * u_cp) =
+                  make_float2(o[0], o[1]);
+            }
+          }
+        }
+        continue;
+      }
 #pragma unroll
       for (int i = 0; i < I_PER_T; ++i)
         if (lds_item[i] >= 0) *reinterpret_cast<f32x4*>(si + lds_item[i]) = rin[k][i];
@@ -322,6 +381,48 @@
     return;
   }
   const float slope = act_slope(a.act);
+  if constexpr (POOL) {
+    constexpr int ES = 36;
+    float* ep = smem + wave * (32 * ES);
+#pragma unroll
+    for (int r = 0; r < 16; ++r) ep[((r & 3) + 8 * (r >> 2) + 4 * lh) * ES + ll] = acc[0][r];
+    __syncthreads();
+    const int ol = tid >> 3, pr = (tid >> 2) & 1, q4 = tid & 3;
+    const int oc = ocg * OCB + ol, oh = a.h >> 1, ow = a.w >> 1;
+    const int opy = (y0 >> 1) + pr, opx = (x0 >> 1) + 4 * q4;
+    if (oc < a.cout && opy < oh && opx < ow) {
+      const float* e0 = smem + (2 * pr) * (32 * ES) + ol * ES + 8 * q4;
+      f32x4 rw[2][2];
+#pragma unroll
+      for (int i = 0; i < 2; ++i)
+#pragma unroll
+        for (int hh = 0; hh < 2; ++hh) rw[i][hh] = *reinterpret_cast<const f32x4*>(e0 + i * (32 * ES) + 4 * hh);
+      const float bb = a.bias ? a.bias[oc] : 0.f;
+#pragma unroll
+      for (int i = 0; i < 2; ++i)
+#pragma unroll
+        for (int hh = 0; hh < 2; ++hh)
+#pragma unroll
+          for (int e = 0; e < 4; ++e) {
+            float q = rw[i][hh][e] + bb;
+            rw[i][hh][e] = (q >= 0.f ? q : q * slope + 0.f) + 0.f;
+          }
+      f32x4 o;
+#pragma unroll
+      for (int j = 0; j < 4; ++j)
+        o[j] = fmaxf(fmaxf(rw[0][j >> 1][2 * (j & 1)], rw[0][j >> 1][2 * (j & 1) + 1]),
+                     fmaxf(rw[1][j >> 1][2 * (j & 1)], rw[1][j >> 1][2 * (j & 1) + 1]));
+      float* yp = a.y + (long long)n * a.y_ns + ((long long)oc * oh + opy) * ow + opx;
+      if (a.vec_ok) {
+        *reinterpret_cast<f32x4*>(yp) = o;
+      } else {
+#pragma unroll
+        for (int j = 0; j < 4; ++j)
+          if (opx + j < ow) yp[j] = o[j];
+      }
+    }
+    return;
+  }
   if (a.vec_ok) {
     constexpr int ES = 36;
     float* ep = smem + (wave % (WM * WN)) * (NT * 32 * ES);
@@ -390,6 +491,15 @@
         if (oc < a.cout && (!(ABL & 4) || v == 12345.678f)) yb[(long long)oc * hw] = v;
       }
   }
+}
+
+template <int WM, int WN, int NT, bool DUAL, int ABL = 0, int KS = 1>
+__global__ __launch_bounds__(WM* WN* KS * 64) void conv3x3_mfma_kernel(Conv3x3Args a) {
+  conv3x3_mfma_body<WM, WN, NT, DUAL, ABL, KS, false, false>(a);
+}
+template <bool DUAL, bool POOL, bool UP2>
+__global__ __launch_bounds__(256, 5) void conv3x3_mfma_glue_kernel(Conv3x3Args a) {
+  conv3x3_mfma_body<4, 1, 1, DUAL, 0, 1, POOL, UP2>(a);
 }
 
 template <bool DUAL>
@@ -692,6 +802,30 @@
   return check_launch("conv3x3_mfma");
 }
 
+static int launch_conv_glue(const Conv3x3Args& a0, int n, bool pool, hipStream_t stream) {
+  Conv3x3Args a = a0;
+  if (pool) {
+    a.vec_ok = ((a.w / 2) % 4 == 0) && ((uintptr_t)a.y % 16 == 0) && (a.y_ns % 4 == 0);
+  } else {
+    a.vec_ok = (a.w % 4 == 0) && ((uintptr_t)a.y % 16 == 0) && (a.y_ns % 4 == 0);
+  }
+  a.tiles_x = cdiv(a.w, TW);
+  a.tiles_y = cdiv(a.h, 4);
+  a.nocg = cdiv(a.cout, 32);
+  a.nchunk = cdiv(a.cin, CK);
+  a.ksplit = 1;
+  const size_t lds = 2 * (size_t)(6 * 2 * RS * 4 + 9 * CK * 32) * sizeof(float);
+  const long long blocks = (long long)a.tiles_x * a.tiles_y * a.nocg * n;
+  TG_REQUIRE(blocks > 0 && blocks < (1ll << 31), TG_E_SHAPE, "conv3x3: grid %lld", blocks);
+  const bool xcd = blocks >= 512;
+  a.nblocks = xcd ? (int)blocks : 0;
+  const unsigned grid = xcd ? (unsigned)(8 * ((blocks + 7) / 8)) : (unsigned)blocks;
+  if (!pool) hipLaunchKernelGGL((conv3x3_mfma_glue_kernel<false, false, true>), dim3(grid), dim3(256), lds, stream, a);
+  else if (a.x2) hipLaunchKernelGGL((conv3x3_mfma_glue_kernel<true, true, false>), dim3(grid), dim3(256), lds, stream, a);
+  else hipLaunchKernelGGL((conv3x3_mfma_glue_kernel<false, true, false>), dim3(grid), dim3(256), lds, stream, a);
+  return check_launch(pool ? "conv3x3_mfma_pool" : "conv3x3_mfma_up2");
+}
+
 __global__ void splitk_finalize_kernel(const float* __restrict__ part, int S, long long part_ss,
                                        const float* __restrict__ bias, float slope, int pool,
                                        float* __restrict__ y, int n, int c, int h, int w) {
@@ -793,7 +927,7 @@
                         const float* res, int64_t res_nstride, float* y, int64_t y_nstride, int n,
                         int cin, int cout, int h, int w, int act, int ksplit, float* partials,
                         tg_stream_t stream, const float* mask = nullptr, int64_t mask_nstride = 0,
-                        int tapsel = 0, int cphase = 0, int set_p0 = 0, int set_p1 = 0) {
+                        int tapsel = 0, int cphase = 0, int set_p0 = 0, int set_p1 = 0, int glue = 0) {
   TG_REQUIRE(x && w_packed && y, TG_E_ARG, "conv3x3_fwd: null pointer");
   TG_REQUIRE(!mask || ksplit <= 1, TG_E_ARG, "conv3x3_fwd: the ReLU mask is applied in the epilogue (no split-K)");
   TG_REQUIRE(n > 0 && cin > 0 && cout > 0 && h > 0 && w > 0, TG_E_SHAPE,
@@ -820,6 +954,7 @@
                "conv3x3: phased taps need 4 phases of %d channels (cin=%d cout=%d)", cphase, cin, cout);
   }
   hipStream_t s = (hipStream_t)stream;
+  if (glue) return launch_conv_glue(a, n, glue == 1, s);
   if (ocb == 32) return launch_conv<4, 1, 1>(a, n, s);
   if (conv3x3_rows_per_wg(ocb, (long long)n * h * w) == 4) return launch_conv<4, 1, 2>(a, n, s);
   if (a.ksplit <= 1 && !tapsel && conv3x3_uses_oneshot(n, cin, cout, h, w)) {
@@ -852,6 +987,24 @@
                               int w, int act, tg_stream_t stream) {
   return conv3x3_impl(x, x_nstride, c1, x2, x2_nstride, w_packed, ocb, bias, res, res_nstride, y,
                       y_nstride, n, cin, cout, h, w, act, 1, nullptr, stream);
+}
+
+extern "C" int tg_conv3x3_glue_supported(int n, int cin, int cout, int h, int w, int ocb, int pool, int up2) {
+  if (n <= 0 || cin <= 0 || cout <= 0 || h < 2 || w < 2 || (h | w) & 1) return 0;
+  if ((pool != 0) == (up2 != 0)) return 0;
+  return ocb == 32 ? 1 : 0;
+}
+
+extern "C" int tg_conv3x3_glue_fwd(const float* x, int64_t x_nstride, int c1, const float* x2, int64_t x2_nstride,
+                                   const float* w_packed, int ocb, const float* bias, float* y, int64_t y_nstride,
+                                   int n, int cin, int cout, int h, int w, int act, int pool, int up2,
+                                   tg_stream_t stream) {
+  TG_REQUIRE(tg_conv3x3_glue_supported(n, cin, cout, h, w, ocb, pool, up2), TG_E_SHAPE,
+             "conv3x3_glue: n=%d cin=%d cout=%d h=%d w=%d ocb=%d pool=%d up2=%d has no folded form "
+             "(tg_conv3x3_glue_supported)", n, cin, cout, h, w, ocb, pool, up2);
+  TG_REQUIRE(!up2 || !x2 || c1 == cin, TG_E_ARG, "conv3x3_glue: the up-sampled input has one source");
+  return conv3x3_impl(x, x_nstride, c1, x2, x2_nstride, w_packed, ocb, bias, nullptr, 0, y, y_nstride, n, cin, cout,
+                      h, w, act, 1, nullptr, stream, nullptr, 0, 0, 0, 0, 0, pool ? 1 : 2);
 }
 
 extern "C" int tg_conv3x3_fwd_phased(const float* x, int64_t x_nstride, const float* w_packed, int ocb,
diff --git a/tecogan-pytorch_amd/csrc/tg_conv3x3_wino.hip b/tecogan-pytorch_amd/csrc/tg_conv3x3_wino.hip
--- a/tecogan-pytorch_amd/csrc/tg_conv3x3_wino.hip
+++ b/tecogan-pytorch_amd/csrc/tg_conv3x3_wino.hip
@@ -95,7 +95,7 @@
   static_assert(PR * RS <= W_ICSTR, "patch of one channel fits the channel stride");
 };
 
-template <bool COH, int TR = 1>
+template <bool COH, int TR = 1, bool POOL = false>
 __device__ __forceinline__ void wino_tile(const WinoArgs& a, int tx, int ty, int ocg, int n) {
   using G = WGeo3<TR>;
   __shared__ __attribute__((aligned(16))) float s_raw[W_ICS * W_ICSTR];
@@ -262,6 +262,24 @@
     }
     if (oc >= a.cout || ox >= a.w) continue;
     const float bz = a.bias ? a.bias[oc] : 0.f;
+    if constexpr (POOL) {
+      if (oy0 + 1 >= a.h || ox + 1 >= a.w) continue;
+      float pv[2][2];
+#pragma unroll
+      for (int i = 0; i < 2; ++i) {
+        float v0 = ((sr[i][0] + sr[i][1]) + sr[i][2]) + bz;
+        float v1 = ((sr[i][1] - sr[i][2]) - sr[i][3]) + bz;
+        if (a.act == TG_ACT_TANH24) { v0 = apply_act(v0, a.act); v1 = apply_act(v1, a.act); }
+        else {
+          v0 = __builtin_fmaxf(v0, slope * v0);
+          v1 = __builtin_fmaxf(v1, slope * v1);
+        }
+        pv[i][0] = v0; pv[i][1] = v1;
+      }
+      st1<COH>(yn + (size_t)oc * ((a.h >> 1) * (a.w >> 1)) + (size_t)(oy0 >> 1) * (a.w >> 1) + (ox >> 1),
+               fmaxf(fmaxf(pv[0][0], pv[0][1]), fmaxf(pv[1][0], pv[1][1])));
+      continue;
+    }
 #pragma unroll
     for (int i = 0; i < 2; ++i) {
       const int oy = oy0 + i;
@@ -302,6 +320,21 @@
   const int ocg = __builtin_amdgcn_readfirstlane(b % a.nocg);
   const int n = __builtin_amdgcn_readfirstlane(b / a.nocg);
   wino_tile<false, TR>(a, tx, ty, ocg, n);
+}
+
+template <int TR>
+__global__ __launch_bounds__(256, 3) void conv3x3_wino_pool_kernel(WinoArgs a) {
+  int b = blockIdx.x;
+  if (a.nblocks > 0) {
+    const int per = (a.nblocks + 7) >> 3;
+    b = (b & 7) * per + (b >> 3);
+    if (b >= a.nblocks) return;
+  }
+  const int tx = __builtin_amdgcn_readfirstlane(b % a.tiles_x); b /= a.tiles_x;
+  const int ty = __builtin_amdgcn_readfirstlane(b % a.tiles_y); b /= a.tiles_y;
+  const int ocg = __builtin_amdgcn_readfirstlane(b % a.nocg);
+  const int n = __builtin_amdgcn_readfirstlane(b / a.nocg);
+  wino_tile<false, TR, true>(a, tx, ty, ocg, n);
 }
 
 struct WinoLayer {
@@ -399,7 +432,7 @@
 int conv3x3_wino_launch(const float* x, int64_t x_ns, int c1, const float* x2, int64_t x2_ns, const float* u,
                         const float* bias, const float* res, int64_t res_ns, const float* mask,
                         int64_t mask_ns, float* y, int64_t y_ns, int n, int cin, int cout, int h, int w,
-                        int act, tg_stream_t stream) {
+                        int act, tg_stream_t stream, bool pool) {
   WinoArgs a{};
   a.x = x; a.x2 = x2; a.u = u; a.bias = bias; a.res = res; a.mask = mask; a.y = y;
   a.x_ns = x_ns; a.x2_ns = x2_ns; a.res_ns = res_ns; a.mask_ns = mask_ns; a.y_ns = y_ns;
@@ -424,6 +457,12 @@
   const bool xcd = xcd_env >= 0 ? xcd_env != 0 : blocks >= 512;
   a.nblocks = xcd ? (int)blocks : 0;
   const unsigned grid = xcd ? (unsigned)(8 * ((blocks + 7) / 8)) : (unsigned)blocks;
+  if (pool) {
+    if (tr == 1) hipLaunchKernelGGL(conv3x3_wino_pool_kernel<1>, dim3(grid), dim3(256), 0, (hipStream_t)stream, a);
+    else if (tr == 2) hipLaunchKernelGGL(conv3x3_wino_pool_kernel<2>, dim3(grid), dim3(256), 0, (hipStream_t)stream, a);
+    else hipLaunchKernelGGL(conv3x3_wino_pool_kernel<4>, dim3(grid), dim3(256), 0, (hipStream_t)stream, a);
+    return check_launch("conv3x3_wino_pool");
+  }
   if (tr == 1) hipLaunchKernelGGL(conv3x3_wino_kernel<1>, dim3(grid), dim3(256), 0, (hipStream_t)stream, a);
   else if (tr == 2) hipLaunchKernelGGL(conv3x3_wino_kernel<2>, dim3(grid), dim3(256), 0, (hipStream_t)stream, a);
   else hipLaunchKernelGGL(conv3x3_wino_kernel<4>, dim3(grid), dim3(256), 0, (hipStream_t)stream, a);
@@ -444,6 +483,23 @@
   TG_REQUIRE((long long)cin * h * w < (1ll << 29), TG_E_SHAPE, "conv3x3_wino: image too large");
   return conv3x3_wino_launch(x, x_nstride, c1, x2, x2_nstride, u_packed, bias, res, res_nstride, relu_mask,
                              mask_nstride, y, y_nstride, n, cin, cout, h, w, act, stream);
+}
+
+extern "C" int tg_conv3x3_wino_pool_supported(int h, int w) { return h >= 2 && w >= 2 ? 1 : 0; }
+
+extern "C" int tg_conv3x3_wino_pool_fwd(const float* x, int64_t x_nstride, int c1, const float* x2,
+                                        int64_t x2_nstride, const float* u_packed, const float* bias, float* y,
+                                        int64_t y_nstride, int n, int cin, int cout, int h, int w, int act,
+                                        tg_stream_t stream) {
+  TG_REQUIRE(x && u_packed && y, TG_E_ARG, "conv3x3_wino_pool: null pointer");
+  TG_REQUIRE(n > 0 && cin > 0 && cout > 0 && h > 0 && w > 0, TG_E_SHAPE, "conv3x3_wino_pool: n=%d cin=%d cout=%d h=%d w=%d",
+             n, cin, cout, h, w);
+  TG_REQUIRE(tg_conv3x3_wino_pool_supported(h, w), TG_E_SHAPE, "conv3x3_wino_pool: h=%d w=%d (>= 2)", h, w);
+  TG_REQUIRE(!x2 || (c1 > 0 && c1 < cin), TG_E_ARG, "conv3x3_wino_pool: c1=%d of cin=%d", c1, cin);
+  TG_REQUIRE(act >= TG_ACT_NONE && act <= TG_ACT_TANH24, TG_E_ARG, "conv3x3_wino_pool: act=%d", act);
+  TG_REQUIRE((long long)cin * h * w < (1ll << 29), TG_E_SHAPE, "conv3x3_wino_pool: image too large");
+  return conv3x3_wino_launch(x, x_nstride, c1, x2, x2_nstride, u_packed, bias, nullptr, 0, nullptr, 0, y, y_nstride, n,
+                             cin, cout, h, w, act, stream, true);
 }
 
 extern "C" int64_t tg_conv3x3_wino_chain_flag_ints(int n_layers, int n, int h, int w) {
diff --git a/tecogan-pytorch_amd/ops.py b/tecogan-pytorch_amd/ops.py
--- a/tecogan-pytorch_amd/ops.py
+++ b/tecogan-pytorch_amd/ops.py
@@ -60,15 +60,15 @@
 
 
 def conv3x3(x, wpk, bias, cin, cout, ocb, act=ACT_NONE, x2=None, res=None, out=None,
-            pool=False, ksplit=None, relu_mask=None):
+            pool=False, ksplit=None, relu_mask=None, up2=False):
     _chk(x, 'x')
     n, c1, h, w = x.shape
     if ksplit is None:
-        ksplit = 1 if (res is not None or relu_mask is not None) else \
+        ksplit = 1 if (res is not None or relu_mask is not None or up2) else \
             L.lib().tg_conv3x3_pick_ksplit(n, cin, cout, h, w)
     if ksplit > 1:
-        if res is not None or relu_mask is not None:
-            raise L.TecoganHipError('conv3x3: split-K path has no residual / mask epilogue')
+        if res is not None or relu_mask is not None or up2:
+            raise L.TecoganHipError('conv3x3: split-K path has no residual / mask epilogue and no up2 input')
         if x2 is not None:
             _chk(x2, 'x2')
         part = torch.empty(ksplit * n * cout * h * w, dtype=torch.float32, device=x.device)
@@ -80,6 +80,10 @@
             wpk.data_ptr(), ocb, _ptr(bias), out.data_ptr(), n, cin, cout, h, w, act, ksplit,
             part.data_ptr(), 1 if pool else 0, _stream()), 'tg_conv3x3_splitk_fwd')
         return out
+    if up2 or (pool and res is None and relu_mask is None and
+               conv3x3_glue_supported(n, cin, cout, h, w, ocb, pool=True)):
+        return _conv3x3_glue(x, wpk, bias, cin, cout, ocb, act, x2, out, pool and not up2, up2,
+                             res is not None or relu_mask is not None or ksplit > 1 or (pool and up2))
     if pool:
         return maxpool2(conv3x3(x, wpk, bias, cin, cout, ocb, act, x2=x2, res=res, ksplit=1))
     if x2 is not None:
@@ -109,6 +113,34 @@
         x.data_ptr(), c1 * hw, c1, _ptr(x2), 0 if x2 is None else x2.shape[1] * hw,
         wpk.data_ptr(), ocb, _ptr(bias), _ptr(res), cout * hw, out.data_ptr(), cout * hw,
         n, cin, cout, h, w, act, _stream()), 'tg_conv3x3_fwd')
+    return out
+
+
+def conv3x3_glue_supported(n, cin, cout, h, w, ocb, pool=False, up2=False):
+    return bool(L.lib().tg_conv3x3_glue_supported(n, cin, cout, h, w, ocb, int(pool), int(up2)))
+
+
+def _conv3x3_glue(x, wpk, bias, cin, cout, ocb, act, x2, out, pool, up2, bad):
+    n, c1, h, w = x.shape
+    if bad:
+        raise L.TecoganHipError('conv3x3: the folded forms take no residual / mask / split-K / pool with up2')
+    if x2 is not None:
+        _chk(x2, 'x2')
+        if x2.shape[0] != n or x2.shape[2:] != x.shape[2:] or c1 + x2.shape[1] != cin:
+            raise L.TecoganHipError(f'conv3x3: x {tuple(x.shape)} x2 {tuple(x2.shape)} cin {cin}')
+    elif c1 != cin:
+        raise L.TecoganHipError(f'conv3x3: x has {c1} channels, weights expect {cin}')
+    ch, cw = (2 * h, 2 * w) if up2 else (h, w)
+    oh, ow = (ch // 2, cw // 2) if pool else (ch, cw)
+    if out is None:
+        out = torch.empty(n, cout, oh, ow, dtype=torch.float32, device=x.device)
+    _chk(out, 'out')
+    if tuple(out.shape) != (n, cout, oh, ow):
+        raise L.TecoganHipError(f'conv3x3: out {tuple(out.shape)}, expected {(n, cout, oh, ow)}')
+    L.check(L.lib().tg_conv3x3_glue_fwd(
+        x.data_ptr(), c1 * h * w, c1, _ptr(x2), 0 if x2 is None else x2.shape[1] * h * w,
+        wpk.data_ptr(), ocb, _ptr(bias), out.data_ptr(), cout * oh * ow,
+        n, cin, cout, ch, cw, act, int(pool), int(up2), _stream()), 'tg_conv3x3_glue_fwd')
     return out
 
 
@@ -1162,7 +1194,11 @@
     return out
 
 
-def conv3x3_wino(x, u_packed, bias, cin, cout, act=ACT_NONE, x2=None, res=None, mask=None, out=None):
+def conv3x3_wino_pool_supported(h, w):
+    return bool(L.lib().tg_conv3x3_wino_pool_supported(h, w))
+
+
+def conv3x3_wino(x, u_packed, bias, cin, cout, act=ACT_NONE, x2=None, res=None, mask=None, out=None, pool=False):
     _chk(x, 'x'); _chk(u_packed, 'u_packed')
     n, c1, h, w = x.shape
     if x2 is not None:
@@ -1170,6 +1206,16 @@
         assert c1 + x2.shape[1] == cin
     else:
         assert c1 == cin
+    if pool:
+        if res is not None or mask is not None:
+            raise L.TecoganHipError('conv3x3_wino: the pooled epilogue takes no residual / mask')
+        y = out if out is not None else torch.empty(n, cout, h // 2, w // 2, dtype=torch.float32, device=x.device)
+        _chk(y, 'out')
+        L.check(L.lib().tg_conv3x3_wino_pool_fwd(
+            x.data_ptr(), x.stride(0), c1, _ptr(x2), x2.stride(0) if x2 is not None else 0,
+            u_packed.data_ptr(), _ptr(bias), y.data_ptr(), y.stride(0), n, cin, cout, h, w, act, _stream()),
+            'tg_conv3x3_wino_pool_fwd')
+        return y
     y = out if out is not None else torch.empty(n, cout, h, w, dtype=torch.float32, device=x.device)
     L.check(L.lib().tg_conv3x3_wino_fwd(
         x.data_ptr(), x.stride(0), c1, _ptr(x2), x2.stride(0) if x2 is not None else 0,
```
